# mfalt/FirstOrderSolvers.jl

Measured on AMD Instinct MI355X. Metric: GAP/DR outer iterations/sec (+ achieved HBM GB/s of the CG SpMV in `roofline`), higher is better.
Workload: dtype f64

## Files before the change

### firstordersolvers.jl_amd/_lib.py

```python
from __future__ import annotations

import ctypes as C
import os
from pathlib import Path

import numpy as np

_HERE = Path(__file__).resolve().parent
LIB_PATH = Path(os.environ["FOSHIP_LIB"]) if os.environ.get("FOSHIP_LIB") else _HERE / "csrc" / "libfoship.so"

FOS_OK = 0
CONE_CODES = {"Free": 0, "Zero": 1, "NonNeg": 2, "NonPos": 3, "SOC": 4, "SOCRotated": 5, "SDP": 6,
              "ExpPrimal": 7, "ExpDual": 8}
SET_CODES = {"IndFree": 0, "IndBallL2": 1, "IndBallL1": 2, "IndSimplex": 3, "IndHalfspace": 4, "IndHyperslab": 5, "IndPoint": 6, "IndBox": 7}
FN_CODES = {"NormL1": 32, "SqrNormL2": 33, "ElasticNet": 34, "Linear": 35, "NormL2": 36, "HuberLoss": 37, "NormLinf": 38}
LS_FORM_CODES = {"sparse_factored": 0, "normal": 1}
ALG_GAP, ALG_GAPA, ALG_FISTA, ALG_DYKSTRA = 0, 1, 2, 3
CG_REFERENCE, CG_FUSED_P, CG_MERGED_SWEEP, CG_MERGED_UPDATE, CG_RESIDENT = 0, 1, 2, 3, 4
DEBUG_PUPDATE_DELAY = 1
STATUS_NAMES = {0: "Continue", 1: "Optimal", 2: "Unbounded", 3: "Infeasible"}


class FosError(RuntimeError):
    def __init__(self, code, msg):
# ... 16 lines not shown
PROTOTYPES = {
    "fos_abi_version": (C.c_int, []),
    "fos_last_error": (C.c_char_p, []),
    "fos_device_count": (C.c_int, [_i32p]),
    "fos_device_name": (C.c_int, [C.c_int, C.c_char_p, C.c_int]),
    "fos_create": (C.c_int, [C.c_int64, C.c_int64, _i64p, _i64p, _dp, _dp, _dp,
                             C.c_int64, _i32p, _i64p, _i64p, C.c_int64, _i32p, _i64p, _i64p, C.c_int, C.POINTER(_h)]),
    "fos_create2": (C.c_int, [C.c_int64, C.c_int64, _i64p, _i64p, _dp, _dp, _dp,
                              C.c_int64, _i32p, _i64p, _i64p, C.c_int64, _i32p, _i64p, _i64p, C.c_int, C.c_int32, C.POINTER(_h)]),
    "fos_create3": (C.c_int, [C.c_int64, C.c_int64, _i64p, _i64p, _dp, _dp, _dp,
                              C.c_int64, _i32p, _i64p, _i64p, C.c_int64, _i32p, _i64p, _i64p, C.c_int, C.c_int32, C.c_int32, C.POINTER(_h)]),
    "fos_get_equilibration": (C.c_int, [_h, _i32p, _dp, _dp, _dp]),
    "fos_host_equilibrate": (C.c_int, [C.c_int64, C.c_int64, _i64p, _i64p, _dp, _dp, _dp,
                                       C.c_int64, _i32p, _i64p, _i64p, C.c_int64, _i32p, _i64p, _i64p, C.c_int32, _dp, _dp, _dp, _dp, _dp, _dp]),
    "fos_destroy": (C.c_int, [_h]),
    "fos_sizes": (C.c_int, [_h, _i64p, _i64p, _i64p, _i64p]),
    "fos_get_cg_total": (C.c_int, [_h, _i64p]),
    "fos_operator_stats": (C.c_int, [_h, _i64p]),
    "fos_comm_get_unique_id": (C.c_int, [C.c_void_p]),
    "fos_set_linesearch": (C.c_int, [_h, C.c_int64]),
    "fos_linesearch_log": (C.c_int, [_h, _dp]),
    "fos_set_longstep": (C.c_int, [_h, C.c_int64, C.c_int64]),
    "fos_longstep_log": (C.c_int, [_h, _dp]),
    "fos_comm_init": (C.c_int, [_h, C.c_int, C.c_int, C.c_void_p]),
    "fos_comm_init_host": (C.c_int, [_h, C.c_int, C.c_int, C.c_void_p, C.c_void_p]),
    "fos_peer_export": (C.c_int, [_h, C.c_void_p]),
    "fos_peer_open": (C.c_int, [_h, C.c_int, C.c_int, C.c_void_p, C.c_double]),
    "fos_peer_open_host": (C.c_int, [_h, C.c_int, C.c_int, C.c_char_p, C.c_double]),
    "fos_peer_close": (C.c_int, [_h]),
    "fos_peer_selftest": (C.c_int, [_h, C.c_int, C.POINTER(C.c_int32)]),
    "fos_exchange_bench": (C.c_int, [_h, C.c_int, _dp]),
    "fos_peer_vec_export": (C.c_int, [_h, C.c_void_p]),
    "fos_peer_vec_open": (C.c_int, [_h, C.c_void_p]),
    "fos_peer_enable": (C.c_int, [_h, C.c_int32]),
    "fos_set_alg": (C.c_int, [_h, C.c_int, C.c_double, C.c_double, C.c_double, C.c_double]),
    "fos_reset_affine": (C.c_int, [_h]),
    "fos_enable_direct": (C.c_int, [_h, _i64p, _i64p, _dp]),
    "fos_disable_direct": (C.c_int, [_h]),
    "fos_get_direct_mode": (C.c_int, [_h, _i32p]),
    "fos_enable_direct2": (C.c_int, [_h, _i64p, _i64p, _dp, C.c_int32]),
    "fos_get_direct_stats": (C.c_int, [_h, _dp]),
    "fos_enable_direct3": (C.c_int, [_h, _i64p, _i64p, _dp, C.c_int32, C.c_int32]),
    "fos_get_direct_stats2": (C.c_int, [_h, _dp]),
    "fos_dense_spd_inverse": (C.c_int, [C.c_int32, C.c_int64, _dp, _dp, C.c_int32, _dp]),
    "fos_host_chol_inverse": (C.c_int, [C.c_int64, _dp, _dp, _i64p]),
    "fos_host_reduced_symm": (C.c_int, [C.c_int64, _dp, _dp, _dp, _i32p]),
    "fos_set_iterate": (C.c_int, [_h, _dp]),
    "fos_get_iterate": (C.c_int, [_h, _dp]),
    "fos_get_checked": (C.c_int, [_h, _dp]),
    "fos_step": (C.c_int, [_h, C.c_int64, C.c_int64, C.c_int64, C.c_double, _i64p, _i32p, C.POINTER(CheckResult)]),
    "fos_getsol": (C.c_int, [_h, _dp, C.c_int32, C.c_double, C.POINTER(CheckResult)]),
    "fos_get_affine_state": (C.c_int, [_h, _dp, _i64p, _i32p]),
    "fos_set_affine_state": (C.c_int, [_h, _dp, C.c_int64]),
    "fos_get_alg_state": (C.c_int, [_h, _dp, _dp, _dp]),
    "fos_set_alg_state": (C.c_int, [_h, _dp, _dp, _dp]),
    "fos_get_cgiter": (C.c_int, [_h, _i64p]),
    "fos_get_alpha12": (C.c_int, [_h, _dp]),
    "fos_get_prox_count": (C.c_int, [_h, _i64p]),
    "fos_q_apply": (C.c_int, [_h, _dp, _dp, C.c_int32]),
    "fos_kkt_apply": (C.c_int, [_h, _dp, _dp]),
    "fos_cg_kkt": (C.c_int, [_h, _dp, _dp, C.c_double, C.c_int64, _i64p]),
    "fos_prox_affine": (C.c_int, [_h, _dp, _dp]),
    "fos_hsdematrix_prox": (C.c_int, [_h, _dp, _dp]),
    "fos_prox_cones": (C.c_int, [_h, _dp, _dp]),
    "fos_check": (C.c_int, [_h, _dp, C.c_double, C.POINTER(CheckResult)]),
    "fos_profile": (C.c_int, [_h, C.c_int32]),
    "fos_profile_read": (C.c_int, [_h, _i64p, _dp, _dp]),
    "fos_profile_read_classes": (C.c_int, [_h, _i64p, _dp]),
    "fos_bench_cg_chain": (C.c_int, [_h, C.c_int32, C.c_int32, C.c_int32, _dp]),
    "fos_bench_kkt": (C.c_int, [_h, C.c_int32, _dp]),
    "fos_psd_debug": (C.c_int, [_h, C.c_int32, C.c_int32]),
    "fos_psd_stats": (C.c_int, [_h, _i32p, C.c_int64, _i64p]),
    "fos_psd_fused_steps": (C.c_int, [_h, _i64p]),
    "fos_sync": (C.c_int, [_h]),
    "fos_host_stacked_spmv": (C.c_int, [C.c_int64, C.c_int64, _i64p, _i64p, _dp, _dp, _dp, C.c_int32, C.c_int32, _i64p]),
    "fos_host_resident_cg": (C.c_int, [C.c_int64, C.c_int64, _i64p, _i64p, _dp, _dp, _dp, C.c_int32, _dp, _dp, C.c_double, C.c_int64, _i64p, _i64p]),
    "fos_host_resident_plan": (C.c_int, [C.c_int64, C.c_int64, _i64p, _i64p, _dp, C.c_int32, _i64p, _i32p, C.c_int64, _i64p, C.c_int64]),
    "fos_host_stacked_spmv_mode": (C.c_int, [C.c_int64, C.c_int64, _i64p, _i64p, _dp, _dp, _dp, C.c_int32, _i64p]),
    "fos_window_stats": (C.c_int, [_h, _i64p]),
    "fos_set_tuning": (C.c_int, [_h, C.c_int32, C.c_int32, C.c_int32]),
    "fos_set_cg_variant": (C.c_int, [_h, C.c_int32]),
    "fos_get_cg_variant": (C.c_int, [_h, _i32p]),
    "fos_resident_stats": (C.c_int, [_h, _i64p]),
    "fos_debug_set": (C.c_int, [_h, C.c_int32, C.c_int64]),
    "fos_set_gapp": (C.c_int, [_h, C.c_int64]),
    "fos_gapp_log": (C.c_int, [_h, _dp]),
    "fos_feas_create": (C.c_int, [C.c_int64, C.c_int32, C.POINTER(_h)]),
    "fos_feas_destroy": (C.c_int, [_h]),
    "fos_feas_set_affine": (C.c_int, [_h, C.c_int32, C.c_int64, _dp, _dp]),
    "fos_feas_set_affine_sparse": (C.c_int, [_h, C.c_int32, C.c_int64, _i64p, _i64p, _dp, _dp]),
    "fos_feas_affine_stats": (C.c_int, [_h, C.c_int32, _dp]),
    "fos_feas_set_affine_factored": (C.c_int, [_h, C.c_int32, C.c_int64, _dp, _dp, C.c_int32, C.c_int32]),
    "fos_feas_affine_factored_stats": (C.c_int, [_h, C.c_int32, _dp]),
    "fos_feas_affine_factored_plan": (C.c_int, [_h, C.c_int32, _i64p]),
    "fos_host_affine_factored": (C.c_int, [C.c_int64, C.c_int64, _dp, _dp, C.c_int32, _dp, _dp]),
    "fos_feas_set_least_squares": (C.c_int, [_h, C.c_int32, C.c_int64, _dp, _dp, C.c_double, C.c_int32]),
    "fos_host_least_squares": (C.c_int, [C.c_int64, C.c_int64, _dp, _dp, C.c_double, _dp, _dp]),
    "fos_feas_set_affine_sparse_factored": (C.c_int, [_h, C.c_int32, C.c_int64, _i64p, _i64p, _dp, _dp, C.c_int32, C.c_int32]),
    "fos_feas_affine_sparse_factored_stats": (C.c_int, [_h, C.c_int32, _dp]),
    "fos_feas_affine_sparse_factored_plan": (C.c_int, [_h, C.c_int32, _i64p]),
    "fos_host_affine_sparse_factored": (C.c_int, [C.c_int64, C.c_int64, _i64p, _i64p, _dp, _dp, C.c_int32, _dp, _dp]),
    "fos_feas_set_quadratic": (C.c_int, [_h, C.c_int32, _dp, _dp, C.c_int32]),
    "fos_feas_set_least_squares_normal": (C.c_int, [_h, C.c_int32, C.c_int64, _dp, _dp, C.c_double, C.c_int32]),
    "fos_feas_set_least_squares_sparse": (C.c_int, [_h, C.c_int32, C.c_int64, _i64p, _i64p, _dp, _dp, C.c_double, C.c_int32, C.c_int32]),
    "fos_feas_nspace_stats": (C.c_int, [_h, C.c_int32, _dp]),
    "fos_host_quadratic": (C.c_int, [C.c_int64, _dp, _dp, _dp, _dp]),
    "fos_host_least_squares_normal": (C.c_int, [C.c_int64, C.c_int64, _dp, _dp, C.c_double, _dp, _dp]),
    "fos_host_least_squares_sparse": (C.c_int, [C.c_int64, C.c_int64, _i64p, _i64p, _dp, _dp, C.c_double, C.c_int32, _dp, _dp]),
    "fos_host_symv_packed": (C.c_int, [C.c_int64, _dp, _dp, _dp, _i32p]),
    "fos_feas_set_quadratic_sparse": (C.c_int, [_h, C.c_int32, _i64p, _i64p, _dp, _dp, C.c_double]),
    "fos_feas_set_least_squares_cg": (C.c_int, [_h, C.c_int32, C.c_int64, _i64p, _i64p, _dp, _dp, C.c_double, C.c_double]),
    "fos_feas_nspace_cg_stats": (C.c_int, [_h, C.c_int32, _dp]),
    "fos_host_quadratic_cg": (C.c_int, [C.c_int64, _i64p, _i64p, _dp, _dp, C.c_double, _dp, _dp, _i32p]),
    "fos_host_least_squares_cg": (C.c_int, [C.c_int64, C.c_int64, _i64p, _i64p, _dp, _dp, C.c_double, C.c_double, _dp, _dp, _i32p]),
    "fos_bench_symv_packed": (C.c_int, [C.c_int32, C.c_int64, C.c_int32, _dp]),
    "fos_feas_set_box": (C.c_int, [_h, C.c_int32, C.c_double, C.c_double]),
    "fos_feas_set_box_arrays": (C.c_int, [_h, C.c_int32, _dp, _dp]),
    "fos_feas_set_cones": (C.c_int, [_h, C.c_int32, C.c_int64, _i32p, _i64p]),
    "fos_feas_set_callback": (C.c_int, [_h, C.c_int32, C.c_void_p, C.c_void_p]),
    "fos_feas_set_blocks": (C.c_int, [_h, C.c_int32, C.c_int64, _i32p, _i64p, _dp, _dp]),
    "fos_feas_set_stats": (C.c_int, [_h, C.c_int32, _dp]),
    "fos_host_set_project": (C.c_int, [C.c_int32, C.c_int64, _dp, _dp, _dp, _dp, _i32p]),
    "fos_feas_set_alg": (C.c_int, [_h, C.c_int32, C.c_double, C.c_double, C.c_double, C.c_double]),
    "fos_feas_set_gapp": (C.c_int, [_h, C.c_double, C.c_double, C.c_double, C.c_int64]),
    "fos_feas_gapp_log": (C.c_int, [_h, _dp]),
    "fos_feas_set_linesearch": (C.c_int, [_h, C.c_int64]),
    "fos_feas_linesearch_log": (C.c_int, [_h, _dp]),
    "fos_feas_set_longstep": (C.c_int, [_h, C.c_int64, C.c_int64]),
    "fos_feas_longstep_log": (C.c_int, [_h, _dp]),
    "fos_feas_set_iterate": (C.c_int, [_h, _dp]),
    "fos_feas_step": (C.c_int, [_h, C.c_int64, C.c_int64, C.c_int64, C.c_double, _i64p, _i32p, _dp, _i32p]),
    "fos_feas_getsol": (C.c_int, [_h, _dp, C.c_int32, C.c_double, _i32p, _dp]),
    "fos_feas_get_iterate": (C.c_int, [_h, _dp]),
    "fos_feas_prox": (C.c_int, [_h, C.c_int32, _dp, _dp]),
    "fos_feas_info": (C.c_int, [_h, _dp, _i32p, _dp]),
}

_lib = None


def load(check_symbols=False):
    global _lib
    if _lib is not None and not check_symbols:
        return _lib
    if not LIB_PATH.exists():
        raise FosError(-100, "%s not found: build it with `make -C %s` (hipcc, gfx950); there is no CPU fallback"
                       % (LIB_PATH, LIB_PATH.parent))
    lib = C.CDLL(str(LIB_PATH), mode=getattr(os, "RTLD_NOW", 2) | getattr(os, "RTLD_GLOBAL", 0x100))
    for name, (res, args) in PROTOTYPES.items():
        fn = getattr(lib, name)
        fn.restype = res
        fn.argtypes = args
    if lib.fos_abi_version() != 1:
        raise FosError(-101, "ABI version mismatch")
    _lib = lib
    return lib


ALLREDUCE_FN = C.CFUNCTYPE(C.c_int, C.c_void_p, C.POINTER(C.c_double), C.c_int64)


def header_symbols():
    import re
    text = (_HERE.parent / "include" / "foship.h").read_text()
    text = re.sub(r"/\*.*?\*/", "", text, flags=re.S)
    return sorted(set(re.findall(r"\b(fos_[a-z0-9_]+)\s*\(", text)))
# ... 24 lines not shown
```

### firstordersolvers.jl_amd/csrc/fos_internal.hpp

```cpp
#pragma once

#include <hip/hip_runtime.h>

#include <algorithm>
#include <cstddef>
#include <cstdint>
#include <cstdio>
#include <cstring>
#include <string>
#include <vector>

#include "foship.h"

namespace fos {

void set_error(const char* fmt, ...);

#define FOS_HIP(expr)                                                                         \
    do {                                                                                      \
        hipError_t _e = (expr);                                                               \
        if (_e != hipSuccess) {                                                               \
            ::fos::set_error("%s:%d: %s -> %s", __FILE__, __LINE__, #expr, hipGetErrorString(_e)); \
            return FOS_EHIP;                                                                  \
        }                                                                                     \
// ... 244 lines not shown
    const PeerBox* fold;
    uint32_t seq_base;
    int32_t batch_mark = 0;
};
constexpr int CGM_RR_STRIDE = 1024;
void launch_cgm_sweep(const LaunchCtx& c, const CgmIter& it, int closes);
void launch_cgm_update(const LaunchCtx& c, const CgmIter& it, bool close_only);
void launch_cgm_apply(const LaunchCtx& c, const CgmIter& it, const double2* v);
void launch_cgm_start(const LaunchCtx& c, const CgmIter& it, const double2* rhs, const double2* v, double tol, int maxit,
                      double2* p_out = nullptr);

struct ResWG { int32_t blk0, nblk, c0, tc, T, wg0, wpu, idx; };
constexpr int RES_GMAX = 512;
constexpr int RES_WPU_MAX = 16;
constexpr int RES_SLOTS = 21;
constexpr int RS_GMAX = 256;
constexpr int RS_WPU_MAX = 4;
constexpr int RS_NCOMP = 7;
constexpr int RS_NTC = 6;
constexpr int RS_NTC_BASE = 3;
constexpr int RS_COMM_LEAD = 2;
inline int rs_ntc(int tmax) { return tmax > 32 ? RS_NTC_BASE : RS_NTC; }
__host__ __device__ inline void rs_split(uint32_t deal, int w, int& t0, int& cnt) {
    t0 = 0;
    for (int k = 0; k < w; ++k) t0 += (int)((deal >> (4 * k)) & 15u);
    cnt = (int)((deal >> (4 * w)) & 15u);
}
inline uint32_t rs_pack(const int (&cnt)[RS_NCOMP + 1]) {
    uint32_t deal = 0;
    for (int w = 0; w <= RS_NCOMP; ++w) deal |= (uint32_t)cnt[w] << (4 * w);
    return deal;
}
inline uint32_t rs_deal(int nblk, int ntc = RS_NTC) {
    int kc = std::min(nblk % RS_NCOMP, RS_NTC_BASE);
    for (int k = std::min(ntc, RS_NTC); k > kc; --k)
        if (k <= (nblk - k + RS_NCOMP - 1) / RS_NCOMP - RS_COMM_LEAD) { kc = k; break; }
    const int per = (nblk - kc) / RS_NCOMP, rem = (nblk - kc) % RS_NCOMP;
    int cnt[RS_NCOMP + 1];
    for (int w = 0; w < RS_NCOMP; ++w) cnt[w] = per + (w < rem ? 1 : 0);
    cnt[RS_NCOMP] = kc;
    return rs_pack(cnt);
}
inline bool rs_deal_ok(uint32_t deal, int nblk, int nt_cap, int ntc) {
    int sum = 0;
    bool gap = false;
    for (int w = 0, t0, cnt; w <= RS_NCOMP; ++w) {
        rs_split(deal, w, t0, cnt);
        if (cnt > (w < RS_NCOMP ? nt_cap : ntc)) return false;
        if (w < RS_NCOMP && cnt > 0 && gap) return false;
        if (cnt == 0) gap = true;
        sum += cnt;
    }
    return sum == nblk;
}
inline int rs_deal_nt(uint32_t deal) {
    int nt = 0;
    for (int w = 0, t0, cnt; w < RS_NCOMP; ++w) { rs_split(deal, w, t0, cnt); nt = std::max(nt, cnt); }
    return nt;
}
constexpr size_t RES_LDS_BUDGET = 160 * 1024;
constexpr size_t RS_STATIC_LDS_MAX = 2560;
inline size_t res_stream_lds_bytes(int tiles) {
    return (size_t)(RS_NCOMP + 1) * 64 * sizeof(double2) + (size_t)4 * RS_GMAX * sizeof(double) + (size_t)(RS_WPU_MAX - 1) * 64 * 2 * sizeof(double) +
           (size_t)tiles * 128 * sizeof(double2);
}
inline size_t res_reg_lds_bytes(int nslot, int tmax) {
    return (size_t)nslot * 64 * 4 * sizeof(double2) + (size_t)nslot * tmax * sizeof(double2) + (size_t)(RES_WPU_MAX - 1) * tmax * 2 * sizeof(double) +
           (size_t)4 * RES_GMAX * sizeof(double);
}
struct ResPlan {
    int G = 0, nw = 0, ncomm = 0, rpt = 0, tmax = 0, tiles_wg_max = 0, units = 0;
    int stream = 0, nt = 0;
    std::vector<ResWG> wg;
    std::string why;
};
bool build_resident_plan(const HostBlkCsr& S, int64_t m, int64_t n, int gmax, ResPlan* out);
int host_resident_cg(const HostBlkCsr& S, const ResPlan& P, int64_t m, int64_t n, const double* cb, double2* x, const double2* rhs, const double2* v0,
                     double tol, int maxit, int* iters);
struct ResLaunch {
    const ResWG* wg; int G, nw, ncomm, rpt, tmax, stream, nt, tiles_wg_max;
    unsigned long long* grec;
    unsigned long long* crec;
    int64_t timeout_ticks;
};
hipError_t launch_cg_resident(const LaunchCtx& c, const ResLaunch& rl, double2* x, const double2* rhs, const double2* v, double tol, int maxit,
                              const PeerBox* fold, uint32_t seq_base);
bool res_lds_fits(const ResLaunch& rl, int device, std::string* why);

enum QMode { Q_PLAIN = 0, Q_RHS = 1, Q_STATUS = 2, Q_VFROMU = 3, Q_PLAIN_NOTAU = 4 };
void launch_q1(const LaunchCtx& c, QMode mode, const double2* v, int comp, double sign, void* out);
void launch_q1_finalize(const LaunchCtx& c, QMode mode, const double2* v, int comp, double sign, void* out, int from_reduced);

void launch_cg_init(const LaunchCtx& c, const double2* rhs, const double2* Ap, double2* r, double2* p);
void launch_cg_init_finalize(const LaunchCtx& c, const double2* r, double tol, int maxit, int from_reduced);
void launch_reduce1(const LaunchCtx& c, int count, int nacc, int gate, int off = 0);
void launch_peer_chain(const LaunchCtx& c, int rounds);

constexpr int LONG_KMAX_ROWS = 32;
struct LongPlanes {
    int64_t interval = 0, nsave = 0;
    int64_t savepos = 0;
    bool now = false;
    double2* P = nullptr;
    double* bpart = nullptr;
    double* dots = nullptr;
    double* nu = nullptr;
    double log[8] = {0};
    int64_t max_supports = 4096;
};
struct LaunchCtx;
void long_save_plane(const LaunchCtx& c, LongPlanes& lp, int which, const double2* y, const double2* x);
int long_project_planes(const LaunchCtx& c, LongPlanes& lp, double2* X, int64_t i);
void launch_long_plane(const LaunchCtx& c, double2* row, const double2* x, const double2* y, double* bpart);
void launch_long_dots(const LaunchCtx& c, const double2* P, int K, int a, const double2* x, double* out);
void launch_long_apply(const LaunchCtx& c, double2* x, const double2* P, int K, const double* nu);
void launch_normdiff(const LaunchCtx& c, const double2* x, const double2* y);
void launch_shift_part2(const LaunchCtx& c, double2* out, const double2* y, const double2* x);
void launch_axpby(const LaunchCtx& c, double2* out, double a, const double2* x, double b, const double2* y);
void launch_relax_a12(const LaunchCtx& c, double2* out, const double2* y, const double2* x);
void launch_gap_final(const LaunchCtx& c, double2* x, const double2* t2, const double2* t1, double alpha, double alpha2,
                      double2* shift_out = nullptr, const double2* sol = nullptr);
void launch_gapa_final(const LaunchCtx& c, double2* x, const double2* t2, const double2* t1, double alpha,
                       double2* shift_out = nullptr, const double2* sol = nullptr);
void launch_gapa_finalize(const LaunchCtx& c, double beta, int from_reduced);
void launch_fista_extrap(const LaunchCtx& c, double2* y, const double2* x, const double2* xold, double coef);
void launch_add(const LaunchCtx& c, double2* out, const double2* a, const double2* b);
void launch_copy(const LaunchCtx& c, double2* out, const double2* in);
void launch_dykstra_corr(const LaunchCtx& c, double2* p, const double2* x, const double2* y);

void launch_dense_q_fill(const LaunchCtx& c, const int64_t* colptr, const int64_t* rowval, const double* nzval, double* Q, int64_t ld);
void launch_dense_gemm(const LaunchCtx& c, int L, double alpha, const double* A, const double* B, double gamma, const double* D, double* Cm);
void launch_dense_resid(const LaunchCtx& c, int64_t L, const double* Y, double* partials, int nblocks);
void launch_dense_scale_identity(const LaunchCtx& c, int64_t L, double* X, double s);
void launch_dense_symv(const LaunchCtx& c, int64_t ld, const double* G, const double* t, double* w);
void launch_dense_spd_inverse_chol(const LaunchCtx& c, int64_t L, const double* G, double* X, double* Lw, double* Ww, int32_t* info);
int64_t host_chol_inverse(int64_t k, const double* K, double* X, bool fused = false);
void launch_dense_gram_rows(const LaunchCtx& c, int64_t m, int64_t ld, const double* A, int64_t L, double* G);
void launch_direct_rhs(const LaunchCtx& c, const double2* W, const double2* x, double* t);
void launch_direct_finish(const LaunchCtx& c, const double2* x, const double2* W, double2* out);

constexpr int RED_TR = 64, RED_TC = 32;
constexpr int RED_TILE = RED_TR * RED_TC;
constexpr int RED_CHUNK = 16;
constexpr int RED_DOT_BLOCKS = 1024;
struct RedUnit { int32_t j, i0, i1, tile0; };
struct RedPlan {
    int64_t k = 0, ntiles = 0;
    int nt = 0, ns = 0;
    std::vector<RedUnit> units;
    std::vector<int32_t> strip_u0;
};
struct RedDev {
    int64_t k, kpad; int nt, nunits;
    const RedUnit* units; const int32_t* strip_u0;
    double* tiles;
    double2* rowslot;
    double* colslot;
};
void build_reduced_plan(int64_t k, RedPlan* P);
void host_reduced_pack(const RedPlan& P, const double* X, std::vector<double>* tiles, int32_t* count);
void host_reduced_symm(const RedPlan& P, const std::vector<double>& tiles, const double* pq, double* y);
void launch_red_form_k(const LaunchCtx& c, int64_t k, int64_t ld, const int32_t* cptr, const int32_t* cidx, const double* cval, const int32_t* rptr,
                       const int32_t* ridx, const double* rval, double* K);
void launch_red_pack_tiles(const LaunchCtx& c, const RedDev& R, int64_t ld, const double* X);
void launch_red_symm(const LaunchCtx& c, const RedDev& R, const double2* pq, double2* y);
void launch_red_in1(const LaunchCtx& c, int swap, const double* t, double2* vin);
void launch_red_pair(const LaunchCtx& c, const RedDev& R, int swap, const double* t, const double* s1, double2* pq);
// ... 230 lines not shown
```

### firstordersolvers.jl_amd/csrc/fos_solver.hpp

```cpp
#pragma once

#include <rccl/rccl.h>

#include <algorithm>

#include "fos_internal.hpp"

typedef double2 d2;

enum DirectForm : int32_t { DIRECT_OFF = 0, DIRECT_DENSE = 1, DIRECT_BLOCK = 2, DIRECT_CG = 3, DIRECT_REDUCED = 4 };

struct DenseInv {
    int used = FOS_DIRECT_FACTOR_NEWTON;
    int steps = 0;
    double seconds = 0.0, probe = 0.0;
    bool fell_back = false;
    int64_t bad_col = -1;
};

enum ReduceVia { VIA_NONE, VIA_RCCL, VIA_HOST, VIA_PEER };
struct HostSeg {
    void* p = nullptr;
    int fd = -1;
    size_t bytes = 0;
    std::string name;
    bool creator = false;
    volatile unsigned long long* ids() const { return reinterpret_cast<volatile unsigned long long*>(static_cast<char*>(p) + bytes - 4096); }
};
struct Transport {
    ncclComm_t comm = nullptr;
    fos_allreduce_fn host_fn = nullptr; void* host_user = nullptr;
    double* host_buf = nullptr;
    unsigned long long* peer_mbox = nullptr;
    unsigned long long* peer_relay = nullptr;
    std::vector<void*> peer_opened;
    fos::PeerBox peer{};
    bool peer_on{false};
    bool peer_same_device = false;
    HostSeg host_seg;
    double* vec_buf = nullptr;
    std::vector<void*> vec_opened;
    fos::VecBox vec{};
    uint32_t vec_seq = 0;
    ReduceVia via() const { return peer_on ? VIA_PEER : (host_fn ? VIA_HOST : (comm ? VIA_RCCL : VIA_NONE)); }
};

struct Operator {
    fos::HostBlkCsr host;
    fos::DevBlkCsr dev{};
    int32_t* wave_blk0 = nullptr; fos::BlkDesc* wave_first = nullptr;
    uint32_t* def_mask = nullptr;
    int64_t win_stats[4] = {0, 0, 0, 0};
    int nwg_target = 2048;
    double* slots_rd = nullptr;
    fos::DefRow* cmp_rec = nullptr; int32_t* cmp_idx = nullptr; double* cmp_local = nullptr; int cmp_lpr = 1;
    fos::ResPlan res_plan;
    fos::ResLaunch res{};
    fos::ResWG* res_wg = nullptr;
    bool res_ok = false;
    bool res_all = false;
    int res_gmax = 0;
};

struct fos_solver {
    int device = 0;
    hipStream_t stream = nullptr;
    int64_t m = 0, n = 0, l = 0, nnz = 0;
    int64_t l_global = 0;

    Operator op;
    std::vector<void*> owned;
    std::vector<void*> pooled;
    double* cb = nullptr;
    double nb = 0.0, nc = 0.0;
    double nb_local = 0.0, nc_local = 0.0;

    d2 *X = nullptr, *T1 = nullptr, *T2 = nullptr;
    d2 *SOL = nullptr, *RHS = nullptr, *R = nullptr, *AP = nullptr;
    d2 *PB[2] = {nullptr, nullptr};
    d2 *Y = nullptr, *XOLD = nullptr;
    d2 *W = nullptr;
    d2 *SOL2 = nullptr;
    double* plain = nullptr;

    fos::ConeSet* cones = nullptr;
    int cus = 256;
    bool psd_fuse = true;
    bool relax_ew = true;

    fos::DevState* st = nullptr;
    fos::DevState* st_host = nullptr;
    fos::HostMark* mark = nullptr;
    double* pre_sums = nullptr;
    bool pre_on = true;
    bool speculate = true;
    double* partials = nullptr;
    double* reduced = nullptr;
    int vec_blocks = 0;
    int cg_blocks = 0;
    bool fuse_p = false;
    int cg_variant = -1;

    int alg = FOS_ALG_GAP;
    double alpha = 0.8, alpha1 = 1.8, alpha2 = 1.8, beta = 0.0;
    double fista_t = 1.0;

    DirectForm direct_form = DIRECT_OFF;
    bool direct_exact() const { return direct_form != DIRECT_OFF && direct_form != DIRECT_CG; }
    double* Ginv = nullptr;
    int64_t Gld = 0;
    int direct_factor_req = 0;
    DenseInv direct_inv;
    double* dvec[2] = {nullptr, nullptr};
    int blk_n = 0;
    int64_t* blk_goff = nullptr;
    int32_t* blk_ioff = nullptr;
    int32_t* blk_idx = nullptr;
    double* blk_ginv = nullptr;
    d2 *blk_phg = nullptr, *blk_qphg = nullptr;
    double* blk_prm = nullptr;
    double* blk_ctx = nullptr;
    bool blk_skip_tail = true;
    bool blk_ready = false;
    bool red_ready = false;
    int red_swap = 0;
    int red_refine = 1;
    fos::RedPlan red_plan;
    fos::RedDev red{};
    d2 *red_pq = nullptr, *red_yk = nullptr;
    double *red_s = nullptr, *red_d = nullptr, *red_r = nullptr, *red_z = nullptr;
    double *red_p = nullptr, *red_q = nullptr, *red_g = nullptr;
    double* red_dots = nullptr;
    double red_minv[4] = {0, 0, 0, 0};
    double direct_setup_s = 0.0;

    int64_t prox_i = 1;
    bool firstrun = true;
    int64_t cgiter = 0;
    int hit_max_accum = 0;
    bool firstrun2 = true;
    int last_cg_pred = 0;
    bool shift_ready = false;
    bool shift_fuse = true;
    bool in_step = false;
    int64_t ls_interval = 0;
    bool ls_now = false;
    int64_t gapp_iproj = 0;
    bool gapp_now = false;
    double gapp_log[23] = {0};
    double ls_log[34] = {0};
    fos::LongPlanes lp;
    int cg_same_run = 0;
    const d2* last_checked = nullptr;

    Transport tr;
    int nranks = 1, rank = 0;
    uint32_t cg_epoch = 0;
    bool sharded() const { return tr.via() != VIA_NONE; }
    bool row_sharded = false;

    int eq_passes = 0;
    std::vector<double> eq_D, eq_E;
    double eq_sigma = 1.0, eq_rho = 1.0, eq_gamma = 1.0;
    double eq_nb = 0.0, eq_nc = 0.0;
    d2* eq_up = nullptr;
    double *eq_inv = nullptr, *eq_cb = nullptr, *eq_w = nullptr;
    bool equilibrated() const { return eq_passes > 0; }

    int cg_chunk = 8;
    bool prof = false;
    int prof_period = 1;
    int64_t cg_total = 0;
    int64_t direct_sweeps = 0;
    struct ProfRec { hipEvent_t a, b; int cls; int j; };
    std::vector<ProfRec> prof_recs;
    size_t prof_used = 0;
    int64_t prof_seen[FOS_PROF_CLASSES] = {0, 0, 0, 0, 0};
    int64_t prof_steps = 0, prof_steps_sampled = 0;
    bool prof_step_on = false;
    static constexpr size_t PROF_CAP = 16384;

    static int sum_slots_over_ranks(void* self);

    fos::LaunchCtx ctx(bool mailboxes = false) const {
        fos::LaunchCtx c;
        c.stream = stream; c.S = op.dev; c.cb = cb; c.n = n; c.m = m; c.l = l; c.st = st;
        c.partials = partials; c.reduced = reduced; c.vec_blocks = vec_blocks; c.cg_blocks = cg_blocks;
        c.peer = (tr.peer_on || mailboxes) ? &tr.peer : nullptr;
        c.def_mask = op.def_mask;
        c.pre = pre_on ? pre_sums : nullptr;
        c.between = nullptr; c.between_arg = nullptr;
        c.cus = cus;
        c.psd_refine_max_mats = (tr.peer_same_device && nranks > 1) ? std::max(1, cus / nranks) : 0;
        c.count_repl = (!row_sharded || rank == 0) ? 1 : 0;
        c.n_repl = row_sharded ? n : 0;
        if (row_sharded) { c.between = &fos_solver::sum_slots_over_ranks; c.between_arg = const_cast<fos_solver*>(this); }
        return c;
    }
};

namespace fos {
int allreduce(fos_solver* h, int count);
int finish_reduce(fos_solver* h, const LaunchCtx& c, int count, int nacc, int gate, int* from_reduced, int off = 0);
void transport_teardown(fos_solver* h, bool destroy = false);
bool peer_fold_env(), peer_loopback_env();
int global_setup(fos_solver* h);
int uncached_acquire(int device, size_t bytes, bool allow_plain, void** out, const char* what);
struct RoctxRange {
    bool on;
    explicit RoctxRange(const char* name);
    ~RoctxRange();
};
int check_launch(const char* where);
int prof_begin(fos_solver* h, int cls, int j, int64_t ordinal);
int prof_begin_other(fos_solver* h, int post);
void prof_end(fos_solver* h, int idx);
int poll_state(fos_solver* h);
int kkt_apply_full(fos_solver* h, const LaunchCtx& c, const d2* w, d2* out, bool deferred = true, bool tau_row = true);
int operator_setup(fos_solver* h, const int64_t* colptr, const int64_t* rowval, const double* nzval);
int operator_repartition(fos_solver* h, int nwg);
int resident_setup(fos_solver* h, int gmax);
int prox_affine_direct(fos_solver* h, const d2* x);

struct Scratch {
    std::vector<void*> held;
    hipError_t err = hipSuccess;
    Scratch() = default;
    Scratch(const Scratch&) = delete;
    Scratch& operator=(const Scratch&) = delete;
    ~Scratch() { for (void* p : held) (void)hipFree(p); }
    template <class T> T* alloc(size_t count) {
        void* p = nullptr;
        if (err == hipSuccess) err = hipMalloc(&p, sizeof(T) * count);
        if (err != hipSuccess) return nullptr;
        held.push_back(p);
        return static_cast<T*>(p);
    }
};

struct DenseWork {
    LaunchCtx c{};
    int64_t L = 0;
    double *G = nullptr, *B0 = nullptr, *B1 = nullptr, *B2 = nullptr, *v0 = nullptr, *v1 = nullptr, *partials = nullptr;
    void fill(Scratch& s) {
        const size_t L2 = (size_t)L * (size_t)L;
        for (double** b : {&B0, &B1, &B2}) *b = s.alloc<double>(L2);
        for (double** v : {&v0, &v1}) if (!*v) *v = s.alloc<double>((size_t)L);
        if (!partials) partials = s.alloc<double>(256);
    }
};
struct DenseOpts {
    const char *what, *gname;
    int factor;
    bool pivot_fallback;
    double bar = 1e-12;
    int newton_extra = 6;
};
int dense_spd_inverse(const DenseWork& k, const DenseOpts& o, double** Xout, DenseInv* st);
void direct_test_vector(int64_t k, int which, std::vector<double>& v);
int factored_inverse(const DevOwned& own, double lambda, int factor, double bar, hipStream_t stream, int64_t m, int64_t L, double* G, double* Xout, DenseInv* inv);

template <class Owner, class T>
int dev_alloc(Owner* h, T** p, size_t count) {
    void* q = nullptr;
    size_t bytes = std::max<size_t>(count, 1) * sizeof(T);
    hipError_t e = hipMalloc(&q, bytes);
    if (e != hipSuccess) { set_error("hipMalloc(%zu bytes): %s", bytes, hipGetErrorString(e)); return FOS_ENOMEM; }
    h->owned.push_back(q);
    *p = reinterpret_cast<T*>(q);
    return FOS_OK;
}

template <class Owner, class T>
int dev_zeros(Owner* h, T** p, size_t count) {
    FOS_TRY(dev_alloc(h, p, count));
    FOS_HIP(hipMemset(*p, 0, sizeof(T) * count));
    return FOS_OK;
}

template <class T>
void dev_release(fos_solver* h, T** p) {
    if (!*p) return;
    auto it = std::find(h->owned.begin(), h->owned.end(), (void*)*p);
    if (it != h->owned.end()) h->owned.erase(it);
    (void)hipFree(*p);
    *p = nullptr;
}

template <class Owner, class T>
int dev_upload(Owner* h, T** p, const std::vector<T>& v) {
    FOS_TRY(dev_alloc(h, p, v.size()));
    if (!v.empty()) FOS_HIP(hipMemcpy(*p, v.data(), v.size() * sizeof(T), hipMemcpyHostToDevice));
    return FOS_OK;
}

inline double sum_squares(const double* v, int64_t count) {
    double s = 0;
    for (int64_t i = 0; i < count; ++i) s += v[i] * v[i];
    return s;
}
}
```

### firstordersolvers.jl_amd/csrc/operator.cpp

```cpp
#include "fos_solver.hpp"

namespace fos {

static int first_target(int cus, const char* wg_env) {
    return wg_env ? std::max(1, std::min(16384, atoi(wg_env))) : cus * 12;
}

static int build_product_operator(int64_t m, int64_t n, const int64_t* colptr, const int64_t* rowval, const double* nzval, int cus, bool row_sharded,
                                  const char* wg_env, HostBlkCsr* out) {
    return build_stacked_csr(m, n, colptr, rowval, nzval, first_target(cus, wg_env), out, cus * 28, -1, row_sharded, cus * 16);
}

static int choose_sweep_grid(HostBlkCsr& hs, int cus, const char* wg_env) {
    int target = first_target(cus, wg_env);
    if (!hs.wpanel.empty()) {
        int nwg = std::min<int>((int)hs.wpanel.size(), cus * hs.wgeom.wg_per_cu);
        if (wg_env) nwg = std::max(1, std::min<int>(atoi(wg_env), (int)hs.wpanel.size()));
        if (nwg >= 8 && (int)hs.wpanel.size() > nwg) nwg -= nwg % 8;
        hs.nwg = nwg;
    } else if (!wg_env && hs.ntiles > hs.nblk / 2) {
        const int64_t waves_target = (int64_t)target * SPMV_WAVES;
        int64_t per_wave = std::max<int64_t>(1, (hs.nblk + waves_target / 2) / waves_target);
        while ((hs.nblk + SPMV_WAVES * per_wave - 1) / (SPMV_WAVES * per_wave) > 16384) ++per_wave;
        target = (int)((hs.nblk + SPMV_WAVES * per_wave - 1) / (SPMV_WAVES * per_wave));
// ... 77 lines not shown
        FOS_TRY(upload(h, &D.wval, hs.wval));
        FOS_TRY(upload(h, &D.wcol, hs.wcol));
        FOS_TRY(upload(h, &D.wrow, hs.wrow));
        window_stats4(hs, o.win_stats);
        drop(hs.wval); drop(hs.wcol); drop(hs.wrow);
    }
    D.nrows = hs.nrows; D.nnz = hs.nnz; D.nnz_padded = hs.nnz_padded;
    D.dbg_flags = getenv("FOS_DBG_FLAGS") ? atoi(getenv("FOS_DBG_FLAGS")) : 0;
    const double op_bytes = 8.0 * (double)hs.nnz_padded + 4.0 * (double)hs.ncol_stored + 48.0 * (double)hs.nblk;
    D.resident = (hs.wpanel.empty() && hs.ntiles == 0 && op_bytes <= 48e6) ? 1 : 0;
    if (const char* e = getenv("FOS_RESIDENT")) D.resident = atoi(e) != 0 ? 1 : 0;
    D.wave_blk0 = o.wave_blk0; D.wave_first = o.wave_first; D.nblk = hs.nblk; D.nwg = hs.nwg; D.nwaves = hs.nwaves;
    D.ndef = (int32_t)hs.def_rows.size(); D.def_lpr = 1;
    if (D.ndef > 0) {
        int32_t* ddi;
        FOS_TRY(upload(h, &D.row_defer, hs.row_defer));
        FOS_TRY(upload(h, &D.def_rows, hs.def_rows));
        FOS_TRY(upload(h, &D.def_ptr, hs.def_ptr));
        FOS_TRY(dev_upload(h, &ddi, hs.def_idx));
        double avg_list = (double)hs.def_ptr.back() / (double)D.ndef;
        if (!(h->row_sharded && hs.ntiles > 0)) {
            FOS_TRY(upload(h, &D.def_rec, hs.def_rec));
            FOS_TRY(dev_zeros(h, &D.slots, (size_t)2 * hs.nslots));
            D.slots_rd = D.slots; D.def_idx = ddi;
            if (h->row_sharded) {
                FOS_TRY(dev_zeros(h, &o.slots_rd, (size_t)2 * hs.nslots));
                D.slots_rd = o.slots_rd;
            }
        } else {
            const size_t nn = (size_t)h->n;
            if (hs.def_rows.size() < nn || hs.def_rows[nn - 1] != (int32_t)(nn - 1)) { set_error("internal: row-sharded tile operator without all rows of A' deferred"); return FOS_EINVAL; }
            TwoViews v;
            two_views(hs.def_rec, hs.def_idx, hs.def_ptr, nn, &v);
            FOS_TRY(dev_upload(h, &o.cmp_rec, v.cmp_rec));
            o.cmp_idx = ddi; o.cmp_lpr = lanes_per_row(v.cmp_avg);
            FOS_TRY(dev_zeros(h, &o.cmp_local, 2 * nn));
            FOS_TRY(upload(h, &D.def_rec, v.rec));
            FOS_TRY(upload(h, &D.def_idx, v.idx));
            FOS_TRY(dev_zeros(h, &o.slots_rd, 2 * (nn + (size_t)hs.nslots)));
            D.slots_rd = o.slots_rd; D.slots = o.slots_rd + 2 * nn;
            avg_list = v.avg;
        }
        int lpr = lanes_per_row(avg_list);
        if (getenv("FOS_DEF_LPR")) lpr = std::max(1, std::min(64, atoi(getenv("FOS_DEF_LPR"))));
        while (lpr & (lpr - 1)) lpr &= lpr - 1;
        D.def_lpr = lpr;
        D.nwg_def = (int32_t)std::min<int64_t>(DEF_MAX_WG, ((int64_t)D.ndef * lpr + DEF_THREADS - 1) / DEF_THREADS);
        std::vector<uint32_t> mask((size_t)(h->l + 31) / 32 + 1, 0u);
        for (int32_t r : hs.def_rows) mask[(size_t)r >> 5] |= 1u << (r & 31);
        FOS_TRY(dev_upload(h, &o.def_mask, mask));
        drop(hs.row_defer); drop(hs.def_idx);
    }
    set_parts(D);
    drop(hs.val); drop(hs.col); drop(hs.row_rel);
    return FOS_OK;
}

int operator_repartition(fos_solver* h, int nwg) {
    Operator& o = h->op;
    nwg = std::min(nwg, 16384);
    if (o.dev.npanel > 0) {
        o.dev.nwg = std::max(1, std::min<int32_t>(nwg, o.dev.npanel));
    } else {
        FOS_HIP(hipStreamSynchronize(h->stream));
        partition_workgroups(&o.host, nwg);
        FOS_HIP(hipMemcpy(o.wave_blk0, o.host.wave_blk0.data(), o.host.wave_blk0.size() * sizeof(int32_t), hipMemcpyHostToDevice));
        FOS_HIP(hipMemcpy(o.wave_first, o.host.wave_first.data(), o.host.wave_first.size() * sizeof(BlkDesc), hipMemcpyHostToDevice));
        o.dev.nwg = o.host.nwg; o.dev.nwaves = o.host.nwaves; o.nwg_target = nwg;
    }
    set_parts(o.dev);
    return FOS_OK;
}

static ResLaunch plan_launch(const ResPlan& p, ResLaunch rl) {
    rl.G = p.G; rl.nw = p.nw; rl.ncomm = p.ncomm; rl.rpt = p.rpt; rl.tmax = p.tmax; rl.stream = p.stream; rl.nt = p.nt; rl.tiles_wg_max = p.tiles_wg_max;
    return rl;
}

static void plan_stats8(const ResPlan& p, bool ok, bool all, int64_t* stats8) {
    stats8[0] = ok ? 1 : 0; stats8[1] = p.G; stats8[2] = p.nw; stats8[3] = p.stream ? -p.nt : p.rpt; stats8[4] = p.units; stats8[5] = p.tiles_wg_max;
    stats8[6] = p.tmax; stats8[7] = all ? 1 : 0;
}

int resident_setup(fos_solver* h, int gmax) {
    Operator& o = h->op;
    if (const char* e = getenv("FOS_RESIDENT_GMAX")) gmax = std::max(1, std::min(gmax, atoi(e)));
    if (o.res_gmax == gmax) return FOS_OK;
    o.res_gmax = gmax; o.res_ok = false;
    ResPlan plan;
    bool ok = build_resident_plan(o.host, h->m, h->n, gmax, &plan);
    if (ok) {
        std::string why;
        ok = res_lds_fits(plan_launch(plan, ResLaunch{}), h->device, &why);
        if (!ok) { plan.why = why; plan.G = 0; plan.wg.clear(); }
    }
    if (!ok) { o.res_plan = plan; o.res_all = false; return FOS_OK; }
    FOS_HIP(hipStreamSynchronize(h->stream));
    if (!o.res.grec) {
        constexpr size_t b1 = sizeof(unsigned long long) * 2 * RES_GMAX * 8, b2 = sizeof(unsigned long long) * 2 * RES_GMAX * 64 * 4;
        void *q1 = nullptr, *q2 = nullptr;
        FOS_TRY(uncached_acquire(h->device, b1, true, &q1, "resident CG records"));
        h->pooled.push_back(q1);
        FOS_TRY(uncached_acquire(h->device, b2, true, &q2, "resident CG column records"));
        h->pooled.push_back(q2);
        FOS_HIP(hipMemset(q1, 0, b1));
        FOS_HIP(hipMemset(q2, 0, b2));
        o.res.grec = static_cast<unsigned long long*>(q1); o.res.crec = static_cast<unsigned long long*>(q2);
    }
    dev_release(h, &o.res_wg);
    FOS_TRY(dev_upload(h, &o.res_wg, plan.wg));
    o.res.wg = o.res_wg;
    o.res = plan_launch(plan, o.res);
    static const double res_wait_s = getenv("FOS_RESIDENT_WAIT_S") ? atof(getenv("FOS_RESIDENT_WAIT_S")) : 5.0;
    o.res.timeout_ticks = (int64_t)(res_wait_s * 1e8);
    o.res_plan = plan; o.res_ok = true; o.res_all = !h->sharded();
    return FOS_OK;
}

static void format_stats12(const HostBlkCsr& S, int64_t* stats) {
    int64_t nell = 0, nlds = 0, nlong = 0, nrun = 0;
    for (const BlkDesc& d : S.blk) {
        if (d.kind() == BLK_ELL) ++nell; else if (d.kind() == BLK_LDS) ++nlds; else if (d.kind() == BLK_LONG) ++nlong;
        if (d.run()) ++nrun;
    }
    stats[0] = S.nblk; stats[1] = nell; stats[2] = nlds; stats[3] = nlong; stats[4] = nrun;
    stats[5] = S.nnz_padded; stats[6] = S.ncol_stored; stats[7] = S.nwaves;
    stats[8] = S.ntiles; stats[9] = S.nslots; stats[10] = (int64_t)S.def_rows.size(); stats[11] = S.tile_values;
}

}

using namespace fos;

extern "C" {

int fos_operator_stats(fos_handle h, int64_t* stats) {
    if (!h || !stats) { set_error("NULL argument"); return FOS_EINVAL; }
    format_stats12(h->op.host, stats);
    stats[7] = h->op.dev.nwaves; stats[10] = h->op.dev.ndef;
    return FOS_OK;
}

int fos_window_stats(fos_handle h, int64_t* stats4) {
    if (!h || !stats4) { set_error("NULL argument"); return FOS_EINVAL; }
    for (int k = 0; k < 4; ++k) stats4[k] = h->op.win_stats[k];
    return FOS_OK;
}

int fos_resident_stats(fos_handle h, int64_t* stats8) {
    if (!h || !stats8) { set_error("NULL argument"); return FOS_EINVAL; }
    const Operator& o = h->op;
    plan_stats8(o.res_plan, o.res_ok, h->sharded() ? o.res_all : o.res_ok, stats8);
    if (!o.res_ok) set_error("FOS_CG_RESIDENT: %s", o.res_plan.why.empty() ? "no plan" : o.res_plan.why.c_str());
    return FOS_OK;
}

int fos_host_resident_cg(int64_t m, int64_t n, const int64_t* colptr, const int64_t* rowval, const double* nzval, const double* b, const double* c,
                         int32_t gmax, double* x, const double* rhs, double tol, int64_t max_iters, int64_t* iters, int64_t* stats8) {
    if (!colptr || m < 0 || n < 0 || gmax < 1 || (x && (!rhs || !b || !c || max_iters < 1))) { set_error("bad argument"); return FOS_EINVAL; }
    HostBlkCsr S;
    FOS_TRY(build_product_operator(m, n, colptr, rowval, nzval, 256, false, nullptr, &S));
    ResPlan P;
    const bool ok = build_resident_plan(S, m, n, gmax, &P);
    if (stats8) plan_stats8(P, ok, ok, stats8);
    if (!ok) { set_error("FOS_CG_RESIDENT: the operator does not qualify (%s)", P.why.c_str()); return x ? FOS_EUNSUPPORTED : FOS_OK; }
    if (!x) return FOS_OK;
    const int64_t l = n + m + 1;
    std::vector<double> cb((size_t)(n + m));
    for (int64_t j = 0; j < n; ++j) cb[j] = c[j];
    for (int64_t i = 0; i < m; ++i) cb[n + i] = b[i];
    std::vector<double2> xv((size_t)l), rv((size_t)l);
    for (int64_t i = 0; i < l; ++i) { xv[i] = double2{x[i], x[l + i]}; rv[i] = double2{rhs[i], rhs[l + i]}; }
    std::vector<double2> v0(xv);
    int it = 0;
    FOS_TRY(host_resident_cg(S, P, m, n, cb.data(), xv.data(), rv.data(), v0.data(), tol, (int)std::min<int64_t>(max_iters, 1 << 30), &it));
    for (int64_t i = 0; i < l; ++i) { x[i] = xv[i].x; x[l + i] = xv[i].y; }
    if (iters) *iters = it;
    return FOS_OK;
}

int fos_host_resident_plan(int64_t m, int64_t n, const int64_t* colptr, const int64_t* rowval, const double* nzval, int32_t gmax,
                           int64_t* info8, int32_t* wg7, int64_t wg_cap, int64_t* tile5, int64_t tile_cap) {
    if (!colptr || !info8 || m < 0 || n < 0 || gmax < 1) { set_error("bad argument"); return FOS_EINVAL; }
    HostBlkCsr S;
    FOS_TRY(build_product_operator(m, n, colptr, rowval, nzval, 256, false, nullptr, &S));
    ResPlan P;
    const bool ok = build_resident_plan(S, m, n, gmax, &P);
    int64_t ntiles = 0;
    for (const ResWG& w : P.wg) ntiles += w.nblk;
    info8[0] = ok ? (P.stream ? 2 : 1) : 0; info8[1] = P.G; info8[2] = P.nt; info8[3] = P.tmax; info8[4] = P.nw; info8[5] = P.rpt; info8[6] = P.ncomm;
    info8[7] = ntiles;
    if (!ok) { set_error("FOS_CG_RESIDENT: the operator does not qualify (%s)", P.why.c_str()); return FOS_OK; }
    if (wg7 && wg_cap >= P.G)
        for (int q = 0; q < P.G; ++q) {
            const ResWG& w = P.wg[q];
            const int32_t r[7] = {w.blk0, w.nblk, w.c0, w.tc, w.wg0, w.wpu, w.idx};
            memcpy(wg7 + 7 * (size_t)q, r, sizeof(r));
        }
    if (tile5 && tile_cap >= ntiles) {
        int64_t k = 0;
        for (const ResWG& w : P.wg)
            for (int ti = 0; ti < w.nblk; ++ti, ++k) {
                const BlkDesc& d = S.blk[w.blk0 + ti];
                int64_t* t = tile5 + 5 * k;
                t[0] = d.meta[0]; t[1] = d.meta[3]; t[2] = d.steps(); t[3] = d.nrows(); t[4] = d.row0;
            }
    }
    return FOS_OK;
}

int fos_debug_resident_deal(int32_t tiles, int32_t steps, int32_t* cnt8, int64_t* lds_bytes) {
    if (tiles < 0 || steps < 1 || steps > 64 || !cnt8) { set_error("bad argument"); return FOS_EINVAL; }
    const uint32_t deal = rs_deal(tiles, rs_ntc(steps));
    for (int w = 0, t0, cnt; w <= RS_NCOMP; ++w) { rs_split(deal, w, t0, cnt); cnt8[w] = cnt; }
    if (lds_bytes) *lds_bytes = (int64_t)res_stream_lds_bytes(tiles);
    return FOS_OK;
}

int fos_host_stacked_spmv(int64_t m, int64_t n, const int64_t* colptr, const int64_t* rowval, const double* nzval,
                          const double* v, double* out, int32_t spmv_workgroups, int32_t resident_waves, int64_t* stats) {
    if (!colptr || !v || !out || m < 0 || n < 0) { set_error("bad argument"); return FOS_EINVAL; }
    HostBlkCsr S;
    FOS_TRY(build_stacked_csr(m, n, colptr, rowval, nzval, spmv_workgroups > 0 ? spmv_workgroups : 1024, &S, resident_waves));
    std::string why;
    int rc = host_stacked_spmv(S, v, out, &why);
    if (rc != FOS_OK) { set_error("operator format check failed: %s", why.c_str()); return rc; }
    if (stats) format_stats12(S, stats);
    return FOS_OK;
}

int fos_host_stacked_spmv_mode(int64_t m, int64_t n, const int64_t* colptr, const int64_t* rowval, const double* nzval,
                               const double* v, double* out, int32_t window_mode, int64_t* stats16) {
    if (!colptr || !v || !out || m < 0 || n < 0) { set_error("bad argument"); return FOS_EINVAL; }
    HostBlkCsr S;
    const bool rs = getenv("FOS_HOST_SPMV_ROW_SHARDED") && atoi(getenv("FOS_HOST_SPMV_ROW_SHARDED")) != 0;
    FOS_TRY(build_stacked_csr(m, n, colptr, rowval, nzval, 1024, &S, 0, window_mode, rs));
// ... 13 lines not shown
```

### firstordersolvers.jl_amd/csrc/resident.hip

```cpp
#include "dev_common.hpp"

namespace fos {

struct ResArgs {
    d2* x;
    const d2* rhs;
    const d2* v;
    const double* cb;
    int n, nm;
    DevState* st;
    const BlkDesc* blk;
    const double* val;
    const ResWG* wg;
    int G;
    unsigned long long* grec;
    unsigned long long* crec;
    int tmax;
    int ncomp;
    int flags;
    double tol;
    int maxit;
    PeerBox pb;
    uint32_t seq_base;
    long long timeout_ticks;
};

__device__ __forceinline__ void res_st_word(unsigned long long* p, unsigned long long w) { __hip_atomic_store(p, w, __ATOMIC_RELAXED, __HIP_MEMORY_SCOPE_AGENT); }
__device__ __forceinline__ unsigned long long res_ld_word(const unsigned long long* p) { return __hip_atomic_load(p, __ATOMIC_RELAXED, __HIP_MEMORY_SCOPE_AGENT); }
__device__ __forceinline__ void res_publish_half(unsigned long long* p, uint32_t seq, double v, int hh) {
    const unsigned long long bits = (unsigned long long)__double_as_longlong(v);
    res_st_word(p + hh, ((unsigned long long)seq << 32) | (hh ? (bits >> 32) : (bits & 0xFFFFFFFFull)));
}
__device__ __forceinline__ bool res_poll_f64(const unsigned long long* p, uint32_t seq, long long timeout, double& out) {
    const long long t0 = wall_clock64();
    unsigned long long lo, hi;
    bool ok;
    do {
        lo = res_ld_word(p); hi = res_ld_word(p + 1);
        ok = (uint32_t)(lo >> 32) == seq && (uint32_t)(hi >> 32) == seq;
    } while (!ok && (wall_clock64() - t0) < timeout);
    out = __longlong_as_double((long long)((hi << 32) | (lo & 0xFFFFFFFFull)));
    return ok;
}

template <int TMAX>
__device__ __forceinline__ void res_tile(const double (&val)[TMAX], int T, const d2 g, const char* __restrict__ gcol, const int (&xoff)[TILE_GROUP],
                                         d2* __restrict__ colpart, int lane, double& u1, double& u2) {
    u1 = 0.0; u2 = 0.0;
#pragma unroll
    for (int grp = 0; grp < TMAX / TILE_GROUP; ++grp) {
        if (grp * TILE_GROUP < T) {
            double p[TILE_GROUP];
#pragma unroll
            for (int h = 0; h < 2; ++h) {
#pragma unroll
                for (int u = 4 * h; u < 4 * h + 4; ++u) {
                    const d2 xc = *reinterpret_cast<const d2*>(gcol + grp * TILE_GROUP * (int)sizeof(d2) + xoff[u]);
                    u1 += val[grp * TILE_GROUP + u] * xc.x; u2 += val[grp * TILE_GROUP + u] * xc.y;
                    p[u] = val[grp * TILE_GROUP + u] * g.x;
                }
                __builtin_amdgcn_sched_barrier(0);
            }
            const double s1 = tile_colsum8_sorted(p);
            __builtin_amdgcn_sched_barrier(0);
#pragma unroll
            for (int u = 0; u < TILE_GROUP; ++u) p[u] = val[grp * TILE_GROUP + u] * g.y;
            const double s2 = tile_colsum8_sorted(p);
            if (lane < TILE_GROUP) colpart[grp * TILE_GROUP + lane] = make_double2(s1, s2);
            __builtin_amdgcn_sched_barrier(0);
        }
    }
}

#ifdef FOS_RES_STAMPS
__device__ long long g_res_stamps[4 * 16 * 64 * 16];
#define RES_STAMP(ph) do { if (stamp_slot >= 0 && stamp_it < 62 && (threadIdx.x & 63) == 0) { __builtin_amdgcn_sched_barrier(0); g_res_stamps[((size_t)stamp_slot * 64 + stamp_it) * 16 + (ph)] = (long long)__builtin_readcyclecounter(); __builtin_amdgcn_sched_barrier(0); } } while (0)
#define RES_STAMP_CAL(where) do { if (stamp_slot >= 0 && (threadIdx.x & 63) == 0) { g_res_stamps[((size_t)stamp_slot * 64 + (where)) * 16 + 6] = (long long)__builtin_readcyclecounter(); g_res_stamps[((size_t)stamp_slot * 64 + (where)) * 16 + 7] = wall_clock64(); } } while (0)
#define RES_STAMP_NEXT() do { stamp_it += 1; } while (0)
#else
#define RES_STAMP(ph) do { } while (0)
#define RES_STAMP_CAL(where) do { } while (0)
#define RES_STAMP_NEXT() do { } while (0)
#endif

enum ResCtl { RC_ALPHA = 0, RC_BETA, RC_GTX, RC_GTY, RC_STOP, RC_NEAR, RC_COUNT };

__device__ __forceinline__ bool res_peer_fold4(const PeerBox& pb, uint32_t seq, double (&tot)[4], bool first, uint32_t* halves ) {
    const int lane = threadIdx.x & 63;
    const size_t par = (size_t)((((seq >> 11) & 1u) << 1) | (seq & 1u)) * PEER_MAX_RANKS;
    bool bad = false;
    for (int t = lane; t < pb.nranks * 8; t += 64) {
        const int hh = t & 1, v = (t >> 1) & 3, r = t >> 3;
        const double mine_d = v == 0 ? tot[0] : (v == 1 ? tot[1] : (v == 2 ? tot[2] : tot[3]));
        const unsigned long long bits = (unsigned long long)__double_as_longlong(mine_d);
        const uint32_t mine = hh ? (uint32_t)(bits >> 32) : (uint32_t)bits;
        if (r == pb.rank && !pb.loopback) { halves[t] = mine; continue; }
        const size_t off_in = PEER_BOX_WORDS + ((par + r) * PEER_MAX_VALS + v) * 2 + hh;
        if (first) {
            const bool wr = !pb.shared || pb.loopback ? (r != pb.rank || pb.loopback) : (r == (pb.rank == 0 ? 1 : 0));
            if (wr) {
                unsigned long long* dst = pb.box[r] + PEER_BOX_WORDS + ((par + pb.rank) * PEER_MAX_VALS + v) * 2 + hh;
                __hip_atomic_store(dst, ((unsigned long long)seq << 32) | mine, __ATOMIC_RELAXED, __HIP_MEMORY_SCOPE_SYSTEM);
            }
        }
        const bool via_relay = pb.relay != nullptr && !first;
        const unsigned long long* src = via_relay ? pb.relay + off_in : pb.box[pb.rank] + off_in;
        long long t0 = 0;
        unsigned long long w;
        bool ok;
        for (uint32_t spin = 1;; ++spin) {
            w = __hip_atomic_load(src, __ATOMIC_RELAXED, __HIP_MEMORY_SCOPE_SYSTEM);
            ok = (uint32_t)(w >> 32) == seq;
            if (ok) break;
            if ((spin & 255u) == 0u) {
                const long long now = wall_clock64();
                if (t0 == 0) t0 = now;
                else if (now - t0 >= pb.timeout_ticks) break;
            }
        }
        if (!ok) bad = true;
        else if (pb.relay != nullptr && first) __hip_atomic_store(pb.relay + off_in, w, __ATOMIC_RELAXED, __HIP_MEMORY_SCOPE_SYSTEM);
        halves[t] = (uint32_t)w;
    }
    __builtin_amdgcn_fence(__ATOMIC_RELEASE, "wavefront");
    __builtin_amdgcn_wave_barrier();
    __builtin_amdgcn_fence(__ATOMIC_ACQUIRE, "wavefront");
    if (__builtin_amdgcn_ballot_w64(bad) != 0ull) return false;
#pragma unroll
    for (int v = 0; v < 4; ++v) {
        double sacc = 0.0;
        for (int r = 0; r < pb.nranks; ++r) {
            const unsigned long long lo = halves[(r * 4 + v) * 2], hi = halves[(r * 4 + v) * 2 + 1];
            sacc += __longlong_as_double((long long)((hi << 32) | lo));
        }
        tot[v] = sacc;
    }
    __builtin_amdgcn_fence(__ATOMIC_RELEASE, "wavefront");
    __builtin_amdgcn_wave_barrier();
    return true;
}

template <int TMAX, int RPT, int LB>
__global__ __launch_bounds__(LB) void cg_resident_kernel(ResArgs a) {
    __shared__ __attribute__((aligned(16))) d2 s_gcol[TMAX];
    __shared__ double s_red[16][4];
    __shared__ double s_ctl[RC_COUNT];
    __shared__ uint32_t s_halves[PEER_MAX_RANKS * 8];
    __shared__ int s_cnt, s_failed;
    extern __shared__ __attribute__((aligned(16))) double s_dyn[];
    constexpr int NSLOT = (LB / 64) * RPT;
    d2* const s_x = reinterpret_cast<d2*>(s_dyn);
    d2* const s_p = s_x + NSLOT * 64;
    d2* const s_s = s_p + NSLOT * 64;
    d2* const s_w = s_s + NSLOT * 64;
    d2* const s_colpart = s_w + NSLOT * 64;
    double* const s_sib = reinterpret_cast<double*>(s_colpart + NSLOT * TMAX);
    double* const s_all = s_sib + (RES_WPU_MAX - 1) * TMAX * 2;
    const int tid = threadIdx.x, lane = tid & 63;
    const int wv = __builtin_amdgcn_readfirstlane(tid >> 6), nw = (int)(blockDim.x >> 6);
    const int ncomp = a.ncomp, ncomm = nw - ncomp;
    const ResWG me = a.wg[blockIdx.x];
    const int T = me.T, tc = me.tc, c0 = me.c0, nm = a.nm;
    DevState* st = a.st;
#ifdef FOS_RES_STAMPS
    int stamp_slot = -1, stamp_it = 0;
    {
        const int b = (int)blockIdx.x;
        const int wslot = b == 0 ? 0 : (b == 1 ? 1 : (b == a.G / 2 ? 2 : (b == a.G - 1 ? 3 : -1)));
// ... 285 lines not shown
#pragma unroll
                for (int k = 0; k < 4; ++k) {
                    const int si = k < me.idx ? k : k - 1;
                    d2 part = k == me.idx ? cp : (si == 0 ? sv[0] : (si == 1 ? sv[1] : (si == 2 ? sv[2] : sv[3])));
                    if (k >= me.wpu) part = make_double2(0.0, 0.0);
                    t.x += part.x; t.y += part.y;
                }
                for (int k = 4; k < me.wpu; ++k) {
                    d2 part = cp;
                    if (k != me.idx) { const int si = k < me.idx ? k : k - 1; part = sib[(size_t)si * TMAX + lane]; }
                    t.x += part.x; t.y += part.y;
                }
                ctot = t;
            }
            const double q1 = ctot.x + gt.x * cc, q2 = ctot.y + gt.y * cc;
            const d2 cwv = make_double2(cr.x - q2, q1 - cr.y);
            const d2 wt = make_double2(gt.x + tot[3], -tot[2] - gt.y);
            RES_STAMP(12);
            double stopf = failed ? 2.0 : 0.0, alpha = 0.0, beta = 0.0;
            if (!failed) {
                if (i < 0) {
                    cr = make_double2(crhs.x - cwv.x, crhs.y - cwv.y);
                    gt = make_double2(rhst.x - wt.x, rhst.y - wt.y);
                } else {
                    gam = tot[0] + (gt.x * gt.x + gt.y * gt.y);
                    if (i > 0 && (sqrt(gam) <= a.tol || i >= a.maxit)) { iter = i; stopf = 1.0; }
                    else {
                        const double delta = tot[1] + (wt.x * gt.x + wt.y * gt.y);
                        if (i == 0) alpha = gam / delta;
                        else {
                            beta = gam / g_prev;
                            alpha = gam / (delta - beta * gam / a_prev);
                        }
                        g_prev = gam; a_prev = alpha;
                        auto upd = [&](const d2 wi, d2& ri, d2& pi, d2& si, d2& xi) {
                            if (i == 0) { pi = ri; si = wi; }
                            else {
                                pi.x = pi.x * beta + ri.x; pi.y = pi.y * beta + ri.y;
                                si.x = si.x * beta + wi.x; si.y = si.y * beta + wi.y;
                            }
                            xi.x += alpha * pi.x; xi.y += alpha * pi.y;
                            ri.x -= alpha * si.x; ri.y -= alpha * si.y;
                        };
                        if (lane < tc) upd(cwv, cr, cpv, csv, cx);
                        upd(wt, gt, pt, stt, xt);
                    }
                }
            }
            RES_STAMP(13);
            if (stopf == 0.0) {
                colG = (leader && lane < tc) ? cr.x * cr.x + cr.y * cr.y : 0.0;
                if (lane < tc) s_gcol[lane] = cr;
            }
            if (lane == 0) { s_ctl[RC_ALPHA] = alpha; s_ctl[RC_BETA] = beta; s_ctl[RC_GTX] = gt.x; s_ctl[RC_GTY] = gt.y; s_ctl[RC_STOP] = stopf; }
        }
        RES_STAMP(6);
        __syncthreads();
        RES_STAMP(7);
        RES_STAMP_NEXT();
        RES_STAMP(0);
        if (s_ctl[RC_STOP] != 0.0) break;
    }
    RES_STAMP_CAL(62);
    if (c0wave) {
        const bool ok = s_ctl[RC_STOP] == 1.0;
        if (ok && leader && lane < tc) a.x[c0 + lane] = cx;
        if (blockIdx.x == 0 && lane == 0) {
            if (ok) {
                a.x[nm] = xt;
                st->rr = gam;
                cg_signal_stop(st, iter, a.maxit, gam, a.seq_base >> 11);
            } else {
                if (a.pb.nranks > 0) st->xchg_failed = 1;
                st->bar_failed = 1; st->done = 1;
            }
        }
    }
}


#ifndef RS_XC
#define RS_XC 2
#endif
__device__ __forceinline__ void res_tile_plain(const double (&val)[TILE_GROUP], const d2 g, const d2* __restrict__ gcol, d2& u, double (&a1)[TILE_GROUP],
                                               double (&a2)[TILE_GROUP]) {
#pragma unroll
    for (int h = 0; h < TILE_GROUP / RS_XC; ++h) {
        d2 xc[RS_XC];
#pragma unroll
        for (int k = 0; k < RS_XC; ++k) xc[k] = gcol[RS_XC * h + k];
#pragma unroll
        for (int k = 0; k < RS_XC; ++k) {
            const double v = val[RS_XC * h + k];
            u.x += v * xc[k].x; u.y += v * xc[k].y;
            a1[RS_XC * h + k] += v * g.x; a2[RS_XC * h + k] += v * g.y;
        }
        __builtin_amdgcn_sched_barrier(0);
    }
}

__device__ __forceinline__ BlkDesc rs_desc(const BlkDesc* blk, int i) {
    typedef const __attribute__((address_space(4))) int64_t cs64;
    cs64* p = (cs64*)(blk + i);
    const int64_t w3 = p[3], w4 = p[4], w5 = p[5];
    BlkDesc d;
    d.nnz0 = p[0]; d.colpos = p[1]; d.cnt = p[2];
    d.row0 = (int32_t)w3; d.info = (int32_t)(w3 >> 32);
    d.meta[0] = (int32_t)w4; d.meta[1] = (int32_t)(w4 >> 32); d.meta[2] = (int32_t)w5; d.meta[3] = (int32_t)(w5 >> 32);
    return d;
}

__device__ __forceinline__ void rs_request(const ResArgs& a, int blk, int grp, int lane, double (&val)[TILE_GROUP]) {
    const BlkDesc d = rs_desc(a.blk, blk);
    const bool live = TILE_GROUP * grp < d.steps();
    const double* __restrict__ vp = a.val + d.nnz0 + (live ? 64 * TILE_GROUP * grp : 0) + (live ? lane : 0);
#pragma unroll
    for (int t = 0; t < TILE_GROUP; ++t) val[t] = __builtin_nontemporal_load(vp + 64 * t);
}


template <int NT> struct RsRows { d2 rr[NT], ww[NT], xx[NT]; };

template <int NT>
__device__ __forceinline__ void rs_rows_load(const ResArgs& a, int blk_first, int cnt, int lane, RsRows<NT>& R) {
#pragma unroll
    for (int q = 0; q < NT; ++q) {
        R.rr[q] = R.ww[q] = R.xx[q] = make_double2(0.0, 0.0);
        if (q < cnt) {
            const BlkDesc d = rs_desc(a.blk, blk_first + q);
            if (lane < d.nrows()) { R.rr[q] = a.v[d.row0 + lane]; R.xx[q] = a.x[d.row0 + lane]; }
        }
    }
}
template <int NT>
__device__ __forceinline__ void rs_rows_store(const ResArgs& a, int blk_first, int cnt, int lane, const RsRows<NT>& R) {
#pragma unroll
    for (int q = 0; q < NT; ++q) {
        if (q < cnt) {
            const BlkDesc d = rs_desc(a.blk, blk_first + q);
            if (lane < d.nrows()) a.x[d.row0 + lane] = R.xx[q];
        }
    }
}

template <int Q, int NT, int D>
__device__ __forceinline__ void rs_group(const ResArgs& a, int bf, int cnt, int grp, int c0, int lane, const d2* __restrict__ s_gcol, d2* __restrict__ mycol,
                                         RsRows<NT>& R, double (&val)[D][TILE_GROUP], double (&a1)[TILE_GROUP], double (&a2)[TILE_GROUP]) {
    if constexpr (Q < NT) {
        if (Q < cnt) {
            const BlkDesc d = rs_desc(a.blk, bf + Q);
            const int coff = d.meta[0] - c0 + TILE_GROUP * grp;
            const bool in = TILE_GROUP * grp < d.steps();
            if (in) res_tile_plain(val[Q % D], R.rr[Q], s_gcol + coff, R.ww[Q], a1, a2);
            if (Q + D < NT && Q + D < cnt) rs_request(a, bf + Q + D, grp, lane, val[Q % D]);
            else rs_request(a, bf + Q % D, grp + 1, lane, val[Q % D]);
            const bool last = Q + 1 == NT || Q + 1 >= cnt || rs_desc(a.blk, bf + Q + 1).meta[0] != d.meta[0];
            if (in && last) {
                const double s1 = tile_colsum8(a1, lane);
                const double s2 = tile_colsum8(a2, lane);
                if (lane < TILE_GROUP && TILE_GROUP * grp + lane < d.meta[3]) mycol[coff + lane] = make_double2(s1, s2);
#pragma unroll
                for (int u = 0; u < TILE_GROUP; ++u) a1[u] = a2[u] = 0.0;
            }
            rs_group<Q + 1, NT, D>(a, bf, cnt, grp, c0, lane, s_gcol, mycol, R, val, a1, a2);
        }
    }
}

#ifndef RS_RING
#define RS_RING 2
#endif
template <int TMAX, int NT>
__device__ __forceinline__ void rs_sweep(const ResArgs& a, int blk_first, int cnt, int c0, int lane, const d2* __restrict__ s_gcol, const double* s_ctl,
                                         d2* __restrict__ mycol, RsRows<NT>& R, double (&acc)[4], bool early = false,
                                         const double* __restrict__ cbh = nullptr) {
    constexpr int D = NT < RS_RING ? NT : RS_RING;
    if (early) cnt = 0;
    mycol[lane] = make_double2(0.0, 0.0);
    acc[0] = acc[1] = acc[2] = acc[3] = 0.0;
    if (cnt > 0) {
        int tw = 0;
#pragma unroll
        for (int q = 0; q < NT; ++q) { const int t = rs_desc(a.blk, blk_first + (q < cnt ? q : cnt - 1)).steps(); tw = t > tw ? t : tw; }
        const int ngrp = ((tw < TMAX ? tw : TMAX) + TILE_GROUP - 1) / TILE_GROUP;
        double val[D][TILE_GROUP], a1[TILE_GROUP], a2[TILE_GROUP];
#pragma unroll
        for (int s = 0; s < D; ++s) if (s < cnt) rs_request(a, blk_first + s, 0, lane, val[s]);
#pragma unroll
        for (int q = 0; q < NT; ++q) R.ww[q] = make_double2(0.0, 0.0);
#pragma unroll
        for (int u = 0; u < TILE_GROUP; ++u) a1[u] = a2[u] = 0.0;
        for (int grp = 0; grp < ngrp; ++grp) {
            int bf = blk_first;
            asm volatile("" : "+s"(bf));
            rs_group<0, NT, D>(a, bf, cnt, grp, c0, lane, s_gcol, mycol, R, val, a1, a2);
        }
        double cb[NT];
#pragma unroll
        for (int q = 0; q < NT; ++q) {
            cb[q] = 0.0;
            if (cbh) cb[q] = cbh[q];
            else if (q < cnt) {
                const BlkDesc d = rs_desc(a.blk, blk_first + q);
                if (lane < d.nrows()) cb[q] = a.cb[d.row0 + lane];
            }
        }
        const d2 gt = make_double2(s_ctl[RC_GTX], s_ctl[RC_GTY]);
#pragma unroll
        for (int q = 0; q < NT; ++q) {
            if (q < cnt) {
                const bool valid = lane < rs_desc(a.blk, blk_first + q).nrows();
                const d2 gq = R.rr[q];
                const double c = cb[q], u1 = R.ww[q].x, u2 = R.ww[q].y;
                const double q1 = -(u1 - gt.x * c), q2 = -(u2 - gt.y * c);
                d2 w = make_double2(gq.x - q2, q1 - gq.y);
                if (!valid) w = make_double2(0.0, 0.0);
                R.ww[q] = w;
                acc[2] += c * gq.x;
                acc[3] += c * gq.y;
            }
        }
    }
#pragma unroll
    for (int q = 0; q < NT; ++q) {
        acc[0] += R.rr[q].x * R.rr[q].x + R.rr[q].y * R.rr[q].y;
        acc[1] += R.ww[q].x * R.rr[q].x + R.ww[q].y * R.rr[q].y;
    }
    if (early) acc[1] = 0.0;
}

template <int NT>
__device__ __forceinline__ void rs_update(const ResArgs& a, int blk_first, int slot_first, int cnt, int lane, int i, double alpha, double beta,
                                          d2* __restrict__ s_ps, RsRows<NT>& R) {
#pragma unroll
    for (int q = 0; q < NT; ++q) {
        if (q < cnt) {
            const size_t e = (size_t)(slot_first + q) * 128 + lane;
            const d2 w = R.ww[q];
            if (i < 0) {
                const BlkDesc d = a.blk[blk_first + q];
                const d2 rh = lane < d.nrows() ? a.rhs[d.row0 + lane] : make_double2(0.0, 0.0);
                R.rr[q] = make_double2(rh.x - w.x, rh.y - w.y);
            } else {
                d2 pq, sq;
                if (i == 0) { pq = R.rr[q]; sq = w; }
                else {
                    pq = s_ps[e]; sq = s_ps[e + 64];
                    pq.x = pq.x * beta + R.rr[q].x; pq.y = pq.y * beta + R.rr[q].y;
                    sq.x = sq.x * beta + w.x; sq.y = sq.y * beta + w.y;
                }
                R.xx[q].x += alpha * pq.x; R.xx[q].y += alpha * pq.y;
                R.rr[q].x -= alpha * sq.x; R.rr[q].y -= alpha * sq.y;
                s_ps[e] = pq; s_ps[e + 64] = sq;
            }
        }
        if ((q & 1) == 1) __builtin_amdgcn_sched_barrier(0);
    }
}

__device__ __forceinline__ bool rs_poll(const ResArgs& a, const ResWG& me, unsigned long long* grec, size_t par, uint32_t seq, int t, int nthr,
                                        double* __restrict__ s_all, double* __restrict__ s_sib) {
    const int tc = me.tc;
    const int nrec = 4 * a.G, nsib = (me.wpu - 1) * tc * 2;
    const int sleepn = (a.flags >> 8) & 0x7F;
    constexpr int PU = 3;
    bool bad = false;
    for (int base = t; base < nrec + nsib; base += PU * nthr) {
        const unsigned long long* src[PU];
        double* dst[PU];
#pragma unroll
        for (int u = 0; u < PU; ++u) {
            const int idx = base + u * nthr;
            src[u] = nullptr; dst[u] = nullptr;
            if (idx < nrec) {
                const int wg = idx >> 2, kk = idx & 3;
                dst[u] = s_all + (size_t)kk * RS_GMAX + wg;
                src[u] = wg == (int)blockIdx.x ? nullptr : grec + (size_t)wg * 8 + 2 * kk;
            } else if (idx < nrec + nsib) {
                const int j = idx - nrec, comp = j & 1, c = (j >> 1) % tc, si = (j >> 1) / tc;
                const int kk = si < me.idx ? si : si + 1;
                dst[u] = s_sib + ((size_t)si * 64 + c) * 2 + comp;
                src[u] = a.crec + ((par * a.G + (size_t)(me.wg0 + kk)) * (size_t)a.tmax + (size_t)c) * 4 + 2 * comp;
            }
        }
        long long tstart = 0;
        for (uint32_t spin = 1;; ++spin) {
            unsigned long long lo[PU], hi[PU];
#pragma unroll
            for (int u = 0; u < PU; ++u) if (src[u]) { lo[u] = res_ld_word(src[u]); hi[u] = res_ld_word(src[u] + 1); }
            bool pending = false;
#pragma unroll
            for (int u = 0; u < PU; ++u) {
                if (src[u]) {
                    if ((uint32_t)(lo[u] >> 32) == seq && (uint32_t)(hi[u] >> 32) == seq) {
                        *dst[u] = __longlong_as_double((long long)((hi[u] << 32) | (lo[u] & 0xFFFFFFFFull)));
                        src[u] = nullptr;
                    } else pending = true;
                }
            }
            if (!pending) break;
            if ((spin & 255u) == 0u) {
                const long long now = wall_clock64();
                if (tstart == 0) tstart = now;
                else if (now - tstart >= a.timeout_ticks) { bad = true; break; }
            }
            if (sleepn >= 2) __builtin_amdgcn_s_sleep(2); else if (sleepn >= 1) __builtin_amdgcn_s_sleep(1);
        }
    }
    return !bad;
}

template <int TMAX, int NT>
__global__ __launch_bounds__(64 * (RS_NCOMP + 1)) void cg_stream_kernel(ResArgs a) {
    __shared__ __attribute__((aligned(16))) d2 s_gcol[64];
    __shared__ double s_red[16][4];
    __shared__ double s_ctl[RC_COUNT];
    __shared__ uint32_t s_halves[PEER_MAX_RANKS * 8];
    __shared__ int s_cnt, s_failed;
    __shared__ double s_tau[9];
    extern __shared__ __attribute__((aligned(16))) double s_dyn[];
    d2* const s_colpart = reinterpret_cast<d2*>(s_dyn);
    double* const s_all = reinterpret_cast<double*>(s_colpart + (RS_NCOMP + 1) * 64);
    double* const s_sib = s_all + 4 * RS_GMAX;
    d2* const s_ps = reinterpret_cast<d2*>(s_sib + (RS_WPU_MAX - 1) * 64 * 2);
    const int tid = threadIdx.x, lane = tid & 63;
    const int wv = __builtin_amdgcn_readfirstlane(tid >> 6), nw = (int)(blockDim.x >> 6);
    constexpr int ncomp = RS_NCOMP;
    const int ncomm = nw - ncomp;
    const ResWG me = a.wg[blockIdx.x];
    const int tc = me.tc, c0 = me.c0, nm = a.nm;
    DevState* st = a.st;
#ifdef FOS_RES_STAMPS
    int stamp_slot = -1, stamp_it = 0;
    {
        const int b = (int)blockIdx.x;
        const int wslot = b == 0 ? 0 : (b == 1 ? 1 : (b == a.G / 2 ? 2 : (b == a.G - 1 ? 3 : -1)));
        if (wslot >= 0 && wv < 16) stamp_slot = wslot * 16 + wv;
    }
#endif
    if (a.pb.nranks > 0 && st->xchg_failed) return;
    if (tid == 0) { s_cnt = 0; s_failed = 0; }
    RES_STAMP_CAL(63);
#ifdef FOS_RES_STAMPS
    if (stamp_slot >= 0 && lane == 0) g_res_stamps[((size_t)stamp_slot * 64 + 63) * 16 + 5] = (long long)__builtin_amdgcn_s_getreg((31 << 11) | 4);
#endif
    int t0, cnt;
    rs_split((uint32_t)me.T, wv, t0, cnt);

    if (wv < ncomp) {
        RsRows<NT> R;
        rs_rows_load<NT>(a, me.blk0 + t0, cnt, lane, R);
        constexpr bool HOLD_CB = NT <= 9;
        double cbh[NT];
#pragma unroll
        for (int q = 0; q < NT; ++q) {
            cbh[q] = 0.0;
            if (HOLD_CB && q < cnt) {
                const BlkDesc d = rs_desc(a.blk, me.blk0 + t0 + q);
                if (lane < d.nrows()) cbh[q] = a.cb[d.row0 + lane];
            }
        }
        d2* const mycol = s_colpart + wv * 64;
        __syncthreads();
        RES_STAMP(0);
        bool early = false;
        for (int i = -1, xr = 0;; ++xr) {
            double acc[4];
            rs_sweep<TMAX, NT>(a, me.blk0 + t0, cnt, c0, lane, s_gcol, s_ctl, mycol, R, acc, early, HOLD_CB ? cbh : nullptr);
#pragma unroll
            for (int k = 0; k < 4; ++k) {
                const double v = wave_sum(acc[k]);
                if (lane == 0) s_red[wv][k] = v;
            }
            RES_STAMP(1);
            __syncthreads();
            RES_STAMP(2);
            {
                const uint32_t seq = a.seq_base + (uint32_t)(xr + 1);
                const size_t par = (size_t)(seq & 1u);
                if (!rs_poll(a, me, a.grec + par * (size_t)a.G * 8, par, seq, tid, (int)blockDim.x, s_all, s_sib)) s_failed = 1;
                __builtin_amdgcn_fence(__ATOMIC_RELEASE, "workgroup");
                if (lane == 0) __hip_atomic_fetch_add(&s_cnt, 1, __ATOMIC_RELAXED, __HIP_MEMORY_SCOPE_WORKGROUP);
            }
            __syncthreads();
            RES_STAMP(3);
            if (s_ctl[RC_STOP] != 0.0) break;
            if (!early) {
                rs_update<NT>(a, me.blk0 + t0, t0, cnt, lane, i, s_ctl[RC_ALPHA], s_ctl[RC_BETA], s_ps, R);
                early = s_ctl[RC_NEAR] != 0.0;
                ++i;
            } else early = false;
            RES_STAMP(4);
            RES_STAMP_NEXT();
            RES_STAMP(0);
        }
        if (s_ctl[RC_STOP] == 1.0) rs_rows_store<NT>(a, me.blk0 + t0, cnt, lane, R);
        RES_STAMP_CAL(62);
        return;
    }

    const int cw = wv - ncomp, ct = tid - 64 * ncomp;
    const bool c0wave = cw == 0, leader = me.idx == 0;
    d2 cx = make_double2(0.0, 0.0), cpv = cx, csv = cx;
    double cc = 0.0;
    for (int q = ct; q < 4 * RS_GMAX; q += 64 * ncomm) s_all[q] = 0.0;
    for (int q = ct + (ncomp + 1) * 4; q < 16 * 4; q += 64 * ncomm) (&s_red[0][0])[q] = 0.0;
    constexpr int NTC = TMAX > 32 ? RS_NTC_BASE : RS_NTC;
    RsRows<NTC> R;
    rs_rows_load<NTC>(a, me.blk0 + t0, c0wave ? cnt : 0, lane, R);
    d2* const mycol = s_colpart + ncomp * 64;
    if (c0wave) {
        d2 cr = make_double2(0.0, 0.0);
        if (lane < tc) { cr = a.v[c0 + lane]; cx = a.x[c0 + lane]; cc = a.cb[c0 + lane]; }
        s_gcol[lane] = cr;
        const d2 gt = a.v[nm], xt = a.x[nm];
        if (lane == 0) { s_ctl[RC_GTX] = gt.x; s_ctl[RC_GTY] = gt.y; s_ctl[RC_STOP] = 0.0; }
        if (lane == 0) { s_tau[0] = xt.x; s_tau[1] = xt.y; s_tau[2] = s_tau[3] = s_tau[4] = s_tau[5] = s_tau[6] = s_tau[7] = s_tau[8] = 0.0; }
        if (blockIdx.x == 0 && lane == 0) { st->tol = a.tol; st->maxit = a.maxit; st->hit_max = 0; st->rn_old = 0.0; }
    }
    __syncthreads();
    int iter = 0;
    uint32_t nx = 0;
    RES_STAMP(0);
    bool early = false;
    for (int i = -1, xr = 0;; ++xr) {
        const uint32_t seq = a.seq_base + (uint32_t)(xr + 1);
        const size_t par = (size_t)(seq & 1u);
        unsigned long long* grec = a.grec + par * (size_t)a.G * 8;
        nx += 1;
        if (c0wave) {
            double racc[4];
            rs_sweep<TMAX, NTC>(a, me.blk0 + t0, cnt, c0, lane, s_gcol, s_ctl, mycol, R, racc, early);
#pragma unroll
            for (int k = 0; k < 4; ++k) {
                const double v = wave_sum(racc[k]);
                if (lane == 0) s_red[ncomp][k] = v;
            }
        }
        RES_STAMP(14);
        __syncthreads();
        RES_STAMP(1);
        d2 cp = make_double2(0.0, 0.0);
        d2 gt = make_double2(0.0, 0.0), cr = gt, crhs = gt, rhst = gt;
        double colG = 0.0;
        if (c0wave) {
            gt = make_double2(s_ctl[RC_GTX], s_ctl[RC_GTY]);
            cr = s_gcol[lane];
            if (i < 0) { crhs = lane < tc ? a.rhs[c0 + lane] : make_double2(0.0, 0.0); rhst = a.rhs[nm]; }
            {
                double rx = cr.x, ry = cr.y;
                asm volatile("" : "+v"(rx), "+v"(ry));
                colG = (leader && lane < tc) ? rx * rx + ry * ry : 0.0;
            }
            double acc[4] = {0.0, 0.0, 0.0, 0.0};
            {
                d2 o[ncomp + 1];
#pragma unroll
                for (int s = 0; s < ncomp + 1; ++s) o[s] = s_colpart[s * 64 + lane];
#pragma unroll
                for (int s = 0; s < ncomp + 1; ++s) { cp.x += o[s].x; cp.y += o[s].y; }
            }
            if (lane < tc && early) { if (leader) acc[0] = colG; }
            else if (lane < tc) {
                acc[1] = cp.x * cr.y - cp.y * cr.x;
                if (leader) {
                    acc[0] = colG;
                    acc[1] += (cr.x * cr.x - cr.y * cr.y) + cc * (gt.x * cr.y - gt.y * cr.x);
                    acc[2] = cc * cr.x;
                    acc[3] = cc * cr.y;
                }
            }
            double mine[4];
            {
                double rv[12];
                const int k4 = lane & 3;
#pragma unroll
                for (int w = 0; w < 12; ++w) rv[w] = s_red[w][k4];
                double sacc = 0.0;
#pragma unroll
                for (int w = 0; w < 12; ++w) sacc += rv[w];
#pragma unroll
                for (int k = 0; k < 4; ++k) {
                    const int lo = __builtin_amdgcn_readlane(__double2loint(sacc), k), hi = __builtin_amdgcn_readlane(__double2hiint(sacc), k);
                    mine[k] = __hiloint2double(hi, lo) + wave_sum(acc[k]);
                }
            }
            if (i < 0) mine[0] = 0.0;
            if (early) { mine[1] = 0.0; mine[2] = 0.0; mine[3] = 0.0; }
            if (lane < 8) {
                const int k = lane >> 1;
                res_publish_half(grec + (size_t)blockIdx.x * 8 + 2 * k, seq, k == 0 ? mine[0] : (k == 1 ? mine[1] : (k == 2 ? mine[2] : mine[3])), lane & 1);
            }
            if (lane < 4) s_all[(size_t)lane * RS_GMAX + blockIdx.x] = lane == 0 ? mine[0] : (lane == 1 ? mine[1] : (lane == 2 ? mine[2] : mine[3]));
            if (me.wpu > 1 && lane < tc) {
                unsigned long long* p = a.crec + ((par * a.G + blockIdx.x) * (size_t)a.tmax + (size_t)lane) * 4;
                res_publish_half(p, seq, cp.x, 0); res_publish_half(p, seq, cp.x, 1);
                res_publish_half(p + 2, seq, cp.y, 0); res_publish_half(p + 2, seq, cp.y, 1);
            }
        }
        RES_STAMP(2);
        {
            if (!rs_poll(a, me, grec, par, seq, tid, (int)blockDim.x, s_all, s_sib)) s_failed = 1;
            __builtin_amdgcn_fence(__ATOMIC_RELEASE, "workgroup");
            if (lane == 0) __hip_atomic_fetch_add(&s_cnt, 1, __ATOMIC_RELAXED, __HIP_MEMORY_SCOPE_WORKGROUP);
        }
        RES_STAMP(3);
        if (c0wave) {
            {
                long long tstart = 0;
                for (uint32_t spin = 1; __hip_atomic_load(&s_cnt, __ATOMIC_RELAXED, __HIP_MEMORY_SCOPE_WORKGROUP) < (int)(nx * (uint32_t)nw); ++spin) {
                    if ((spin & 4095u) == 0u) {
                        const long long now = wall_clock64();
                        if (tstart == 0) tstart = now;
                        else if (now - tstart >= 2 * a.timeout_ticks) { s_failed = 1; break; }
                    }
                }
                __builtin_amdgcn_fence(__ATOMIC_ACQUIRE, "workgroup");
            }
            RES_STAMP(4);
            bool failed = __hip_atomic_load(&s_failed, __ATOMIC_RELAXED, __HIP_MEMORY_SCOPE_WORKGROUP) != 0;
            d2 xt = make_double2(s_tau[0], s_tau[1]), pt = make_double2(s_tau[2], s_tau[3]), stt = make_double2(s_tau[4], s_tau[5]);
            double g_prev = s_tau[6], a_prev = s_tau[7], gam = s_tau[8];
            double tot[4];
#pragma unroll
            for (int k = 0; k < 4; ++k) {
                double rv[RS_GMAX / 64];
#pragma unroll
                for (int j = 0; j < RS_GMAX / 64; ++j) rv[j] = s_all[(size_t)k * RS_GMAX + lane + 64 * j];
                double sacc = 0.0;
#pragma unroll
                for (int j = 0; j < RS_GMAX / 64; ++j) sacc += rv[j];
                tot[k] = wave_sum(sacc);
            }
            if (!failed && a.pb.nranks > 0) failed = !res_peer_fold4(a.pb, seq, tot, blockIdx.x == 0, s_halves);
            RES_STAMP(5);
            d2 ctot = cp;
            if (me.wpu > 1 && lane < tc) {
                const d2* sib = reinterpret_cast<const d2*>(s_sib);
                d2 t = make_double2(0.0, 0.0);
                for (int kk = 0; kk < me.wpu; ++kk) {
                    d2 part = cp;
                    if (kk != me.idx) part = sib[(size_t)(kk < me.idx ? kk : kk - 1) * 64 + lane];
                    t.x += part.x; t.y += part.y;
                }
                ctot = t;
            }
            const double q1 = ctot.x + gt.x * cc, q2 = ctot.y + gt.y * cc;
            const d2 cwv = make_double2(cr.x - q2, q1 - cr.y);
            const d2 wt = make_double2(gt.x + tot[3], -tot[2] - gt.y);
            double stopf = failed ? 2.0 : 0.0, alpha = 0.0, beta = 0.0, near = 0.0;
            if (!failed && early) {
                gam = tot[0] + (gt.x * gt.x + gt.y * gt.y);
                if (i > 0 && (sqrt(gam) <= a.tol || i >= a.maxit)) { iter = i; stopf = 1.0; }
            } else if (!failed) {
                if (i < 0) {
                    cr = make_double2(crhs.x - cwv.x, crhs.y - cwv.y);
                    gt = make_double2(rhst.x - wt.x, rhst.y - wt.y);
                } else {
                    gam = tot[0] + (gt.x * gt.x + gt.y * gt.y);
                    if (i > 0 && (sqrt(gam) <= a.tol || i >= a.maxit)) { iter = i; stopf = 1.0; }
                    else {
                        const double delta = tot[1] + (wt.x * gt.x + wt.y * gt.y);
                        if (i == 0) alpha = gam / delta;
                        else {
                            beta = gam / g_prev;
                            alpha = gam / (delta - beta * gam / a_prev);
                        }
                        g_prev = gam; a_prev = alpha;
                        auto upd = [&](const d2 wi, d2& ri, d2& pi, d2& si, d2& xi) {
                            if (i == 0) { pi = ri; si = wi; }
                            else {
                                pi.x = pi.x * beta + ri.x; pi.y = pi.y * beta + ri.y;
                                si.x = si.x * beta + wi.x; si.y = si.y * beta + wi.y;
                            }
                            xi.x += alpha * pi.x; xi.y += alpha * pi.y;
                            ri.x -= alpha * si.x; ri.y -= alpha * si.y;
                        };
                        if (lane < tc) upd(cwv, cr, cpv, csv, cx);
                        upd(wt, gt, pt, stt, xt);
                        near = (sqrt(gam) <= 3.0 * a.tol || i + 1 >= a.maxit) ? 1.0 : 0.0;
                    }
                }
            }
            if (stopf == 0.0 && !early) s_gcol[lane] = lane < tc ? cr : make_double2(0.0, 0.0);
            if (lane == 0) {
                if (!early) { s_ctl[RC_ALPHA] = alpha; s_ctl[RC_BETA] = beta; s_ctl[RC_GTX] = gt.x; s_ctl[RC_GTY] = gt.y; s_ctl[RC_NEAR] = near; }
                s_ctl[RC_STOP] = stopf;
                s_tau[0] = xt.x; s_tau[1] = xt.y; s_tau[2] = pt.x; s_tau[3] = pt.y; s_tau[4] = stt.x; s_tau[5] = stt.y; s_tau[6] = g_prev; s_tau[7] = a_prev; s_tau[8] = gam;
            }
        }
        RES_STAMP(6);
        __syncthreads();
        RES_STAMP(7);
        RES_STAMP_NEXT();
        RES_STAMP(0);
        if (s_ctl[RC_STOP] != 0.0) break;
        if (!early) {
            if (c0wave) rs_update<NTC>(a, me.blk0 + t0, t0, cnt, lane, i, s_ctl[RC_ALPHA], s_ctl[RC_BETA], s_ps, R);
            early = s_ctl[RC_NEAR] != 0.0;
            ++i;
        } else early = false;
    }
    RES_STAMP_CAL(62);
    if (c0wave) {
        const bool ok = s_ctl[RC_STOP] == 1.0;
        if (ok) rs_rows_store<NTC>(a, me.blk0 + t0, cnt, lane, R);
        if (ok && leader && lane < tc) a.x[c0 + lane] = cx;
        if (blockIdx.x == 0 && lane == 0) {
            if (ok) {
                a.x[nm] = make_double2(s_tau[0], s_tau[1]);
                const double gam = s_tau[8];
                st->rr = gam;
                cg_signal_stop(st, iter, a.maxit, gam, a.seq_base >> 11);
            } else {
                if (a.pb.nranks > 0) st->xchg_failed = 1;
                st->bar_failed = 1; st->done = 1;
            }
        }
    }
}

struct ResKernel { const void* fn; int threads; size_t lds; };
static ResKernel res_kernel(const ResLaunch& rl) {
    auto k = [](auto kern, int threads, size_t lds) { return ResKernel{reinterpret_cast<const void*>(kern), threads, lds}; };
    if (rl.stream) {
        const int thr = 64 * (RS_NCOMP + 1);
        const size_t lds = res_stream_lds_bytes(rl.tiles_wg_max);
        if (rl.tmax > 32 && rl.nt <= 3) return k(cg_stream_kernel<64, 3>, thr, lds);
        if (rl.tmax > 32) return k(cg_stream_kernel<64, 5>, thr, lds);
        if (rl.nt <= 3) return k(cg_stream_kernel<32, 3>, thr, lds);
        if (rl.nt <= 5) return k(cg_stream_kernel<32, 5>, thr, lds);
        if (rl.nt <= 9) return k(cg_stream_kernel<32, 9>, thr, lds);
        return k(cg_stream_kernel<32, 10>, thr, lds);
    }
    const int thr = 64 * (rl.nw + rl.ncomm);
    if (rl.tmax <= 32 && rl.rpt == 1) return k(cg_resident_kernel<32, 1, 768>, thr, res_reg_lds_bytes(12, 32));
    if (rl.tmax <= 32 && rl.rpt == 2) return k(cg_resident_kernel<32, 2, 512>, thr, res_reg_lds_bytes(16, 32));
    if (rl.tmax <= 32) return k(cg_resident_kernel<32, 3, 512>, thr, res_reg_lds_bytes(24, 32));
    return k(cg_resident_kernel<64, 1, 512>, thr, res_reg_lds_bytes(8, 64));
}

static hipError_t res_lds_optin(const ResKernel& k) {
    if (k.lds > 48 * 1024) return hipFuncSetAttribute(k.fn, hipFuncAttributeMaxDynamicSharedMemorySize, (int)k.lds);
    return hipSuccess;
}

bool res_lds_fits(const ResLaunch& rl, int device, std::string* why) {
    const ResKernel k = res_kernel(rl);
    hipFuncAttributes fa{};
    int cap = 0;
    char buf[192];
    if (hipFuncGetAttributes(&fa, k.fn) != hipSuccess || hipDeviceGetAttribute(&cap, hipDeviceAttributeMaxSharedMemoryPerBlock, device) != hipSuccess) {
        (void)hipGetLastError();
        *why = "the kernel's or the device's LDS size could not be read";
        return false;
    }
    if (k.lds + fa.sharedSizeBytes > (size_t)cap) {
        snprintf(buf, sizeof(buf), "a workgroup's LDS (%zu + %zu static bytes) exceeds the device's %d", k.lds, (size_t)fa.sharedSizeBytes, cap);
        *why = buf;
        return false;
    }
    const hipError_t e = res_lds_optin(k);
    if (e != hipSuccess) {
        (void)hipGetLastError();
        snprintf(buf, sizeof(buf), "the LDS opt-in for %zu bytes failed (%s)", k.lds, hipGetErrorString(e));
        *why = buf;
        return false;
    }
    return true;
}

hipError_t launch_cg_resident(const LaunchCtx& c, const ResLaunch& rl, double2* x, const double2* rhs, const double2* v, double tol, int maxit,
                              const PeerBox* fold, uint32_t seq_base) {
    ResArgs a{};
    a.x = x; a.rhs = rhs; a.v = v; a.cb = c.cb; a.n = (int)c.n; a.nm = (int)(c.n + c.m); a.st = c.st;
    a.blk = c.S.blk; a.val = c.S.val; a.wg = rl.wg; a.G = rl.G; a.grec = rl.grec; a.crec = rl.crec; a.tmax = rl.tmax;
    a.tol = tol; a.maxit = maxit;
    a.pb = fold ? *fold : PeerBox{}; a.seq_base = seq_base;
    a.timeout_ticks = rl.timeout_ticks;
    a.ncomp = rl.nw;
    static const int res_flags = getenv("FOS_RES_FLAGS") ? atoi(getenv("FOS_RES_FLAGS")) : (2 << 8);
    a.flags = res_flags;
    const ResKernel k = res_kernel(rl);
    const hipError_t e = res_lds_optin(k);
    if (e != hipSuccess) return e;
    void* args[] = {&a};
    return hipLaunchKernel(k.fn, dim3(rl.G), dim3(k.threads), args, k.lds, c.stream);
}

}

extern "C" int fos_debug_res_stamps(long long* out, int n) {
#ifdef FOS_RES_STAMPS
    if (n > 4 * 16 * 64 * 16) n = 4 * 16 * 64 * 16;
    return (int)hipMemcpyFromSymbol(out, HIP_SYMBOL(fos::g_res_stamps), sizeof(long long) * (size_t)n);
#else
    (void)out; (void)n; return -1;
#endif
}
```

### firstordersolvers.jl_amd/csrc/solver.cpp

```cpp
#include <dlfcn.h>
#include <functional>

#include <chrono>
#include <cmath>
#include <mutex>

#include "fos_solver.hpp"

namespace fos {
const char* last_error_cstr();

struct Roctx {
    int state = 0;
    int (*push)(const char*) = nullptr;
    int (*pop)() = nullptr;
};
static Roctx g_roctx;
static bool roctx_on() {
    if (g_roctx.state == 0) {
        g_roctx.state = -1;
        const char* e = getenv("FOS_ROCTX");
        if (e && atoi(e) != 0) {
            const char* names[] = {"librocprofiler-sdk-roctx.so", "librocprofiler-sdk-roctx.so.1", "libroctx64.so", "libroctx64.so.4"};
            for (const char* nm : names) {
// ... 125 lines not shown
}

}

using namespace fos;

namespace {

int wait_cg_mark(fos_solver* h, uint32_t epoch, int32_t batch_id, bool* ended) {
    FOS_TRY(check_launch("poll"));
    volatile HostMark* m = h->mark;
    static const double wait_s = getenv("FOS_CG_WAIT_S") ? atof(getenv("FOS_CG_WAIT_S")) : 120.0;
    const auto t0 = std::chrono::steady_clock::now();
    for (uint32_t spin = 1;; ++spin) {
        if (__atomic_load_n(&m->seq, __ATOMIC_ACQUIRE) == epoch) { *ended = true; break; }
        if (__atomic_load_n(&m->batch, __ATOMIC_ACQUIRE) == batch_id) { *ended = false; break; }
        __builtin_ia32_pause();
        if ((spin & 0xFFFFu) == 0 && hipStreamQuery(h->stream) == hipSuccess) {
            if (__atomic_load_n(&m->seq, __ATOMIC_ACQUIRE) == epoch) { *ended = true; break; }
            if (__atomic_load_n(&m->batch, __ATOMIC_ACQUIRE) == batch_id) { *ended = false; break; }
            FOS_TRY(poll_state(h));
            *ended = h->st_host->done != 0;
            return FOS_OK;
        }
        if ((spin & 0xFFFFFu) == 0 && std::chrono::duration<double>(std::chrono::steady_clock::now() - t0).count() > wait_s) {
            set_error("CG solve %u: neither its end mark nor its batch mark arrived within %.0f s (a kernel of the solve does not finish)", epoch, wait_s);
            return FOS_EHIP;
        }
    }
    if (*ended) { h->st_host->done = 1; h->st_host->iter = m->iter; h->st_host->hit_max = m->hit_max; h->st_host->rr = m->rr; }
    else h->st_host->done = 0;
    return FOS_OK;
}

typedef std::function<int(const LaunchCtx&)> PostFn;
int cg_solve(fos_solver* h, d2* x, const d2* rhs, double tol, int maxit, int64_t* iters, const d2* apply_on = nullptr,
             const PostFn* post = nullptr, bool* post_ran = nullptr) {
    LaunchCtx c = h->ctx();
    int next_j = 1;
    const bool fold = h->tr.peer_on && peer_fold_env();
    const bool rccl = h->sharded() && !fold;
    int32_t variant = FOS_CG_REFERENCE;
    FOS_TRY(fos_get_cg_variant(h, &variant));
    const bool resident = variant == FOS_CG_RESIDENT;
    const bool merged = variant == FOS_CG_MERGED_SWEEP || variant == FOS_CG_MERGED_UPDATE;
    const bool close_in_update = variant == FOS_CG_MERGED_UPDATE;
    const bool fuse_p = variant == FOS_CG_FUSED_P;
    static const bool start_env = !(getenv("FOS_CG_FUSED_START") && atoi(getenv("FOS_CG_FUSED_START")) == 0);
    const bool start_fused = !merged && !h->sharded() && !c.between && start_env;
    const uint32_t nwin = (uint32_t)std::min<int64_t>((2 * (int64_t)std::max(maxit, 0) + 4 + 2047) / 2048, (int64_t)1 << 20);
    uint32_t epoch = h->cg_epoch + 1u;
    if (const uint32_t off = epoch & 0x1FFFFFu; off != 0u && off + (nwin - 1u) > 0x1FFFFFu) epoch += 0x200000u - off;
    h->cg_epoch = epoch + (nwin - 1u);
    const uint32_t seq_base = (uint32_t)(epoch * 2048u);
    auto iter_desc = [&](int j) {
        CgIter it;
        it.j = j; it.r = h->R; it.p_prev = h->PB[(j - 1) & 1]; it.p_cur = h->PB[j & 1];
        it.fuse_p = fuse_p; it.rr_from_reduced = rccl ? 1 : 0; it.fold = fold ? &h->tr.peer : nullptr; it.seq_base = seq_base;
        it.start_fused = start_fused;
        return it;
    };
    auto merged_desc = [&](int j) {
        CgmIter it;
        it.j = j; it.x = x; it.r = h->R; it.p = h->PB[0]; it.s = h->PB[1]; it.w = h->AP;
        it.close_in_update = close_in_update; it.from_reduced = rccl ? 1 : 0; it.fold = fold ? &h->tr.peer : nullptr; it.seq_base = seq_base;
        return it;
    };
    const size_t prof_start = h->prof_used;
    const bool spec = post && h->speculate && !c.between && !fuse_p && (seq_base >> 11) != 0u &&
                      (!h->sharded() || (fold && h->alg != FOS_ALG_GAPA));
    const int32_t batch_id = (int32_t)(((seq_base >> 11) & 0x7FFFFFu) << 8 | 1u);
    bool mark_last = spec;
    auto merged_reduce = [&](int j) -> int {
        if (c.between) FOS_TRY(c.between(c.between_arg));
        if (!rccl) return FOS_OK;
        launch_reduce1(c, c.S.nwg, 3, 1, 0);
        LaunchCtx c2 = c;
        c2.partials = c.partials + 3 * (size_t)PART_CAP + (size_t)((j - 1) & 1) * CGM_RR_STRIDE;
        c2.reduced = c.reduced + 3;
        launch_reduce1(c2, c.cg_blocks, 1, 1);
        return allreduce(h, 4);
    };
    if (resident) {
        const int pe = prof_begin(h, FOS_PROF_RESIDENT, 1, h->prof_seen[FOS_PROF_RESIDENT]++);
        const hipError_t le = launch_cg_resident(c, h->op.res, x, rhs, apply_on ? apply_on : x, tol, maxit, fold ? &h->tr.peer : nullptr, seq_base);
        prof_end(h, pe);
        if (le != hipSuccess) { set_error("resident CG launch: %s", hipGetErrorString(le)); return FOS_EHIP; }
        if (spec) {
            LaunchCtx cg = c;
            cg.gate = &h->st->done;
            FOS_TRY((*post)(cg));
            bool ended = false;
            FOS_TRY(wait_cg_mark(h, (uint32_t)(seq_base >> 11), batch_id, &ended));
            if (!ended) { set_error("resident CG solve %u ended without its mark", (unsigned)(seq_base >> 11)); return FOS_EHIP; }
            if (post_ran) *post_ran = true;
        } else {
            FOS_TRY(poll_state(h));
            if (!h->st_host->done) { set_error("resident CG solve %u did not finish", (unsigned)(seq_base >> 11)); return FOS_EHIP; }
        }
        *iters = h->st_host->iter;
        h->cg_same_run = (h->st_host->iter == h->last_cg_pred) ? h->cg_same_run + 1 : 0;
        h->last_cg_pred = h->st_host->iter;
        h->cg_total += h->st_host->iter;
        if (h->st_host->hit_max) h->hit_max_accum = 1;
        return FOS_OK;
    }
    if (merged) {
        CgmIter it0 = merged_desc(0);
        const d2* v = apply_on ? apply_on : x;
        const int po = prof_begin_other(h, 0);
        launch_cgm_apply(c, it0, v);
        if (c.between) FOS_TRY(c.between(c.between_arg));
        if (rccl) { launch_reduce1(c, c.S.nwg, 3, 0, 0); FOS_TRY(allreduce(h, 3)); }
        launch_cgm_start(c, it0, rhs, v, tol, maxit);
        prof_end(h, po);
        const int pe = prof_begin(h, FOS_PROF_KKT, 0, h->cg_total);
        launch_cgm_sweep(c, it0, close_in_update ? -1 : 0);
        prof_end(h, pe);
    } else if (start_fused) {
        CgmIter it0 = merged_desc(0);
        const d2* v = apply_on ? apply_on : x;
        const int po = prof_begin_other(h, 0);
        launch_cgm_apply(c, it0, v);
        launch_cgm_start(c, it0, rhs, v, tol, maxit, h->PB[1]);
        prof_end(h, po);
    } else {
        int fr = 0;
        const int po = prof_begin_other(h, 0);
        FOS_TRY(kkt_apply_full(h, c, apply_on ? apply_on : x, h->AP));
        launch_cg_init(c, rhs, h->AP, h->R, h->PB[1]);
        FOS_TRY(finish_reduce(h, c, c.vec_blocks, 1, 0, &fr));
        launch_cg_init_finalize(c, h->R, tol, maxit, fr);
        prof_end(h, po);
    }
    auto enqueue = [&](int count) -> int {
        if (merged) {
            for (int q = 0; q < count && next_j <= maxit; ++q, ++next_j) {
                CgmIter it = merged_desc(next_j);
                const bool last = q == count - 1 || next_j == maxit;
                if (mark_last && last) it.batch_mark = batch_id;
                FOS_TRY(merged_reduce(next_j));
                int pe = prof_begin(h, FOS_PROF_CGVEC, next_j, (h->cg_total + next_j - 1) % 4 == 1 ? (h->cg_total + next_j - 1) / 4 : 1);
                launch_cgm_update(c, it, false);
                prof_end(h, pe);
                pe = prof_begin(h, FOS_PROF_KKT, next_j + (close_in_update ? 0 : 1), h->cg_total + next_j);
                launch_cgm_sweep(c, it, close_in_update ? -1 : next_j);
                prof_end(h, pe);
            }
            if (close_in_update) {
                CgmIter it = merged_desc(next_j);
                if (mark_last) it.batch_mark = batch_id;
                FOS_TRY(merged_reduce(next_j));
                launch_cgm_update(c, it, true);
            }
            return FOS_OK;
        }
        for (int q = 0; q < count && next_j <= maxit; ++q, ++next_j) {
            CgIter it = iter_desc(next_j);
            if (mark_last && (q == count - 1 || next_j == maxit)) it.batch_mark = batch_id;
            int pe = prof_begin(h, FOS_PROF_KKT, next_j, h->cg_total + next_j - 1);
            launch_kkt2_cg(c, it, h->AP);
            prof_end(h, pe);
            int f1 = 0;
            if (c.between) FOS_TRY(c.between(c.between_arg));
            if (rccl) { launch_reduce1(c, c.S.nwg, 3, 1, 0); FOS_TRY(allreduce(h, 3)); f1 = 1; }
            pe = prof_begin(h, FOS_PROF_CGVEC, next_j, (h->cg_total + next_j - 1) % 4 == 1 ? (h->cg_total + next_j - 1) / 4 : 1);
// ... 635 lines not shown
    FOS_HIP(hipMemcpyAsync(lp.nu, nu2.data(), sizeof(double) * 2 * K, hipMemcpyHostToDevice, c.stream));
    launch_long_apply(c, X, lp.P, K, lp.nu);
    FOS_HIP(hipStreamSynchronize(c.stream));
    lp.log[0] = (double)i; lp.log[1] = (double)best_active; lp.log[2] = (double)best_viol; lp.log[3] = (double)qsqrt(step2 > 0 ? step2 : (qreal)0);
    lp.log[4] = (double)K; lp.log[5] = (double)tried;
    return FOS_OK;
}
void long_save_plane(const LaunchCtx& c, LongPlanes& lp, int which, const d2* y, const d2* x) {
    const int64_t row = 2 * (lp.savepos - 1) + which;
    launch_long_plane(c, lp.P + row * c.l, x, y, lp.bpart + row * c.vec_blocks);
}
}

extern "C" {

int fos_abi_version(void) { return FOS_ABI_VERSION; }
const char* fos_last_error(void) { return fos::last_error_cstr(); }

int fos_device_count(int* count) {
    int n = 0;
    hipError_t e = hipGetDeviceCount(&n);
    if (e != hipSuccess || n <= 0) {
        if (count) *count = 0;
        set_error("no HIP device visible (%s): libfoship has no CPU fallback", e == hipSuccess ? "count = 0" : hipGetErrorString(e));
        return FOS_ENODEVICE;
    }
    if (count) *count = n;
    return FOS_OK;
}

int fos_device_name(int device, char* buf, int buflen) {
    hipDeviceProp_t prop;
    FOS_HIP(hipGetDeviceProperties(&prop, device));
    snprintf(buf, buflen, "%s (%s, %d CUs)", prop.name, prop.gcnArchName, prop.multiProcessorCount);
    return FOS_OK;
}

struct HandleGuard {
    fos_solver* h;
    ~HandleGuard() { if (h) fos_destroy(h); }
};

int fos_create(int64_t m, int64_t n, const int64_t* colptr, const int64_t* rowval, const double* nzval,
               const double* b, const double* c,
               int64_t nK1, const int32_t* K1type, const int64_t* K1start, const int64_t* K1len,
               int64_t nK2, const int32_t* K2type, const int64_t* K2start, const int64_t* K2len,
               int device, fos_handle* out) {
    return fos_create2(m, n, colptr, rowval, nzval, b, c, nK1, K1type, K1start, K1len, nK2, K2type, K2start, K2len, device, 0, out);
}

int fos_create2(int64_t m, int64_t n, const int64_t* colptr, const int64_t* rowval, const double* nzval,
                const double* b, const double* c,
                int64_t nK1, const int32_t* K1type, const int64_t* K1start, const int64_t* K1len,
                int64_t nK2, const int32_t* K2type, const int64_t* K2start, const int64_t* K2len,
                int device, int32_t flags, fos_handle* out) {
    if (!out) { set_error("out handle is NULL"); return FOS_EINVAL; }
    *out = nullptr;
    if (m < 0 || n < 0 || !colptr || (!rowval && colptr[n] > 1) || (!b && m) || (!c && n)) { set_error("NULL or negative argument"); return FOS_EINVAL; }
    int ndev = 0;
    FOS_TRY(fos_device_count(&ndev));
    if (device < 0 || device >= ndev) { set_error("device %d out of range (0..%d)", device, ndev - 1); return FOS_EINVAL; }
    FOS_TRY(cone_table_check("K1", m, nK1, K1type, K1start, K1len));
    FOS_TRY(cone_table_check("K2", n, nK2, K2type, K2start, K2len));
    FOS_HIP(hipSetDevice(device));

    HandleGuard guard{new fos_solver()};
    fos_solver* h = guard.h;
    h->device = device;
    h->m = m; h->n = n; h->l = n + m + 1; h->l_global = h->l;
    h->nnz = colptr[n] - 1;
    FOS_HIP(hipStreamCreateWithFlags(&h->stream, hipStreamNonBlocking));
    FOS_HIP(hipHostMalloc((void**)&h->mark, sizeof(HostMark), hipHostMallocMapped));
    memset(h->mark, 0, sizeof(HostMark));
    h->speculate = !(getenv("FOS_SPECULATE") && atoi(getenv("FOS_SPECULATE")) == 0);
    h->shift_fuse = !(getenv("FOS_SHIFT_FUSE") && atoi(getenv("FOS_SHIFT_FUSE")) == 0);

    hipDeviceProp_t prop;
    FOS_HIP(hipGetDeviceProperties(&prop, device));
    const int cus = prop.multiProcessorCount > 0 ? prop.multiProcessorCount : 256;
    h->cus = cus;
    const PsdTuning psd_tuning = PsdTuning::from_env();
    h->psd_fuse = !(getenv("FOS_PSD_FUSE") && atoi(getenv("FOS_PSD_FUSE")) == 0);
    h->relax_ew = !(getenv("FOS_RELAX_EW") && atoi(getenv("FOS_RELAX_EW")) == 0);

    h->row_sharded = (flags & FOS_CREATE_ROW_SHARDED) != 0;
    FOS_TRY(operator_setup(h, colptr, rowval, nzval));
    h->fuse_p = false;
    if (const char* e = getenv("FOS_CG_FUSE_P")) h->fuse_p = atoi(e) != 0;
    if (const char* e = getenv("FOS_CG_VARIANT")) h->cg_variant = std::max(-1, std::min((int)FOS_CG_RESIDENT, atoi(e)));

    std::vector<double> cbv((size_t)(n + m));
    for (int64_t j = 0; j < n; ++j) { cbv[j] = c[j]; }
    for (int64_t i = 0; i < m; ++i) { cbv[n + i] = b[i]; }
    h->nb = std::sqrt(sum_squares(b, m)); h->nc = std::sqrt(sum_squares(c, n));
    h->nb_local = h->nb; h->nc_local = h->nc;
    FOS_TRY(dev_upload(h, &h->cb, cbv));

    const size_t l = (size_t)h->l;
    d2** vecs[] = {&h->X, &h->T1, &h->T2, &h->SOL, &h->RHS, &h->R, &h->PB[0], &h->PB[1], &h->AP, &h->Y, &h->XOLD, &h->W, &h->SOL2};
    for (d2** v : vecs) FOS_TRY(dev_zeros(h, v, l));
    FOS_TRY(dev_alloc(h, &h->plain, 2 * l));
    h->vec_blocks = (int)std::max<int64_t>(1, std::min<int64_t>((h->l + 255) / 256, 1024));
    h->cg_blocks = std::min(h->vec_blocks, getenv("FOS_CG_BLOCKS") ? std::max(1, atoi(getenv("FOS_CG_BLOCKS"))) : 2 * cus);
    if (h->op.dev.ndef > 0)
        h->cg_blocks = std::max<int>(h->cg_blocks, (int)std::min<int64_t>(1024, ((int64_t)h->op.dev.ndef * h->op.dev.def_lpr + 255) / 256));
    h->cg_blocks = std::min(h->cg_blocks, 1024);

    ConeTable table;
    table.ew.assign(l, 0);
    cone_table_add(table, 0, CONE_K2, nK2, K2type, K2start, K2len);
    cone_table_add(table, n, CONE_K1, nK1, K1type, K1start, K1len);
    table.ew[l - 1] = (uint8_t)(EW_MAX0 | (EW_MAX0 << 2));
    ConeSetOptions cone_opts;
    cone_opts.warm = !getenv("FOS_PSD_COLD");
    cone_opts.refine_records = true;
    cone_opts.debug_rec = getenv("FOS_PSD_DEBUG_REC") != nullptr;
    FOS_TRY(cone_set_build(table, (int64_t)l, cone_opts, psd_tuning, &h->cones));

    FOS_TRY(dev_zeros(h, &h->st, 1));
    FOS_TRY(dev_zeros(h, &h->pre_sums, 128));
    h->pre_on = !(getenv("FOS_CG_PRE") && atoi(getenv("FOS_CG_PRE")) == 0);
    {
        void* dp = nullptr;
        FOS_HIP(hipHostGetDevicePointer(&dp, h->mark, 0));
        const unsigned long long addr = (unsigned long long)(uintptr_t)dp;
        FOS_HIP(hipMemcpy(&h->st->hostmark, &addr, sizeof(addr), hipMemcpyHostToDevice));
    }
    FOS_HIP(hipHostMalloc((void**)&h->st_host, sizeof(DevState), hipHostMallocDefault));
    memset(h->st_host, 0, sizeof(DevState));
    FOS_TRY(dev_alloc(h, &h->partials, (size_t)6 * PART_CAP));
    FOS_TRY(dev_zeros(h, &h->reduced, 16));
    if (const char* e = getenv("FOS_CG_CHUNK")) h->cg_chunk = std::max(1, atoi(e));

    FOS_TRY(resident_setup(h, cus));
    FOS_TRY(fos_set_alg(h, FOS_ALG_GAP, 0.8, 1.8, 1.8, 0.0));
    FOS_TRY(fos_set_iterate(h, nullptr));
    FOS_HIP(hipStreamSynchronize(h->stream));
    *out = h;
    guard.h = nullptr;
    return FOS_OK;
}

int fos_create3(int64_t m, int64_t n, const int64_t* colptr, const int64_t* rowval, const double* nzval,
                const double* b, const double* c,
                int64_t nK1, const int32_t* K1type, const int64_t* K1start, const int64_t* K1len,
                int64_t nK2, const int32_t* K2type, const int64_t* K2start, const int64_t* K2len,
                int device, int32_t flags, int32_t equil_passes, fos_handle* out) {
    if (equil_passes == 0) return fos_create2(m, n, colptr, rowval, nzval, b, c, nK1, K1type, K1start, K1len, nK2, K2type, K2start, K2len, device, flags, out);
    if (!out) { set_error("out handle is NULL"); return FOS_EINVAL; }
    *out = nullptr;
    if (equil_passes < 0 || equil_passes > EQ_MAX_PASSES) { set_error("equil_passes = %d: 0 .. %d", (int)equil_passes, EQ_MAX_PASSES); return FOS_EINVAL; }
    if (flags & FOS_CREATE_ROW_SHARDED) {
        set_error("equilibration needs the whole problem on one handle: a rank knows neither the other ranks' column norms nor the global sigma, rho");
        return FOS_EUNSUPPORTED;
    }
    EqScaling eq;
    FOS_TRY(host_equilibrate(m, n, colptr, rowval, nzval, b, c, nK1, K1type, K1start, K1len, nK2, K2type, K2start, K2len, equil_passes, &eq));
    fos_handle h = nullptr;
    FOS_TRY(fos_create2(m, n, colptr, rowval, eq.nz.data(), eq.b.data(), eq.c.data(), nK1, K1type, K1start, K1len, nK2, K2type, K2start, K2len, device, flags, &h));
    HandleGuard guard{h};
    h->eq_nb = std::sqrt(sum_squares(b, m)); h->eq_nc = std::sqrt(sum_squares(c, n));
    h->eq_sigma = eq.sigma; h->eq_rho = eq.rho; h->eq_gamma = eq.gamma;
    const size_t l = (size_t)h->l;
    std::vector<d2> up(l);
    std::vector<double> inv((size_t)(n + m)), cbv((size_t)(n + m));
    for (int64_t j = 0; j < n; ++j) {
        up[j] = make_double2(eq.sigma / eq.E[j], eq.rho * eq.E[j]);
        inv[j] = 1.0 / eq.E[j];
        cbv[j] = eq.c[j];
    }
    for (int64_t i = 0; i < m; ++i) {
        up[n + i] = make_double2(eq.rho / eq.D[i], eq.sigma * eq.D[i]);
        inv[n + i] = 1.0 / eq.D[i];
        cbv[n + i] = eq.b[i];
    }
    up[l - 1] = make_double2(1.0, eq.sigma * eq.rho);
    for (const d2& u : up)
        if (!(u.x > 0.0) || !(u.y > 0.0) || !std::isfinite(u.x) || !std::isfinite(u.y)) { set_error("equilibration: a scale factor left the range of fp64"); return FOS_EINVAL; }
    FOS_TRY(dev_upload(h, &h->eq_up, up));
    FOS_TRY(dev_upload(h, &h->eq_inv, inv));
    FOS_TRY(dev_upload(h, &h->eq_cb, cbv));
    FOS_TRY(dev_zeros(h, &h->eq_w, l));
    h->eq_D.swap(eq.D);
    h->eq_E.swap(eq.E);
    h->eq_passes = equil_passes;
    *out = h;
    guard.h = nullptr;
    return FOS_OK;
}

int fos_get_equilibration(fos_handle h, int32_t* passes, double* D, double* E, double* scal3) {
    if (!h) { set_error("NULL handle"); return FOS_EINVAL; }
    if (passes) *passes = h->eq_passes;
    if (D) { if (h->equilibrated()) std::copy(h->eq_D.begin(), h->eq_D.end(), D); else std::fill(D, D + h->m, 1.0); }
    if (E) { if (h->equilibrated()) std::copy(h->eq_E.begin(), h->eq_E.end(), E); else std::fill(E, E + h->n, 1.0); }
    if (scal3) { scal3[0] = h->eq_sigma; scal3[1] = h->eq_rho; scal3[2] = h->eq_gamma; }
    return FOS_OK;
}

int fos_destroy(fos_handle h) {
    if (!h) return FOS_OK;
    (void)hipSetDevice(h->device);
    if (h->stream) (void)hipStreamSynchronize(h->stream);
    transport_teardown(h, true);
    for (auto& r : h->prof_recs) { (void)hipEventDestroy(r.a); (void)hipEventDestroy(r.b); }
    cone_set_destroy(h->cones, h->stream);
    for (void* p : h->pooled) uncached_release(p);
    for (void* p : h->owned) (void)hipFree(p);
    if (h->st_host) (void)hipHostFree(h->st_host);
    if (h->mark) (void)hipHostFree(h->mark);
    if (h->stream) (void)hipStreamDestroy(h->stream);
    delete h;
    return FOS_OK;
}

int fos_sizes(fos_handle h, int64_t* m, int64_t* n, int64_t* N, int64_t* nnz) {
    if (!h) { set_error("NULL handle"); return FOS_EINVAL; }
// ... 418 lines not shown
            launch_cgm_apply(c, it, h->W);
            launch_cgm_start(c, it, h->RHS, h->W, -1.0, INT32_MAX);
            launch_cgm_sweep(c, it, it.close_in_update ? -1 : 0);
            for (int j = 1; j <= iters; ++j) {
                it.j = j;
                launch_cgm_update(c, it, false);
                launch_cgm_sweep(c, it, it.close_in_update ? -1 : j);
            }
            return;
        }
        for (int j = 1; j <= iters; ++j) {
            CgIter it;
            it.j = j; it.r = h->R; it.p_prev = h->PB[(j - 1) & 1]; it.p_cur = h->PB[j & 1];
            it.fuse_p = variant == FOS_CG_FUSED_P; it.rr_from_reduced = 0; it.fold = nullptr; it.seq_base = seq_base;
            launch_kkt2_cg(c, it, h->AP);
            launch_cg_update(c, it, h->W, h->R, h->AP, 0);
            if (!it.fuse_p) launch_cg_pupdate(c, it, h->W, h->PB[(j + 1) & 1]);
        }
    };
    hipEvent_t e0, e1;
    FOS_HIP(hipEventCreate(&e0));
    FOS_HIP(hipEventCreate(&e1));
    hipGraph_t graph = nullptr;
    hipGraphExec_t exec = nullptr;
    if (use_graph) {
        FOS_HIP(hipStreamSynchronize(h->stream));
        FOS_HIP(hipStreamBeginCapture(h->stream, hipStreamCaptureModeThreadLocal));
        chain();
        FOS_HIP(hipStreamEndCapture(h->stream, &graph));
        FOS_HIP(hipGraphInstantiate(&exec, graph, nullptr, nullptr, 0));
        FOS_HIP(hipGraphLaunch(exec, h->stream));
    } else {
        chain();
    }
    FOS_HIP(hipEventRecord(e0, h->stream));
    for (int rep = 0; rep < reps; ++rep) {
        if (use_graph) FOS_HIP(hipGraphLaunch(exec, h->stream));
        else chain();
    }
    FOS_HIP(hipEventRecord(e1, h->stream));
    FOS_HIP(hipEventSynchronize(e1));
    float ms = 0.f;
    FOS_HIP(hipEventElapsedTime(&ms, e0, e1));
    *ms_per_iter = (double)ms / ((double)reps * iters);
    if (exec) (void)hipGraphExecDestroy(exec);
    if (graph) (void)hipGraphDestroy(graph);
    (void)hipEventDestroy(e0);
    (void)hipEventDestroy(e1);
    FOS_TRY(check_launch("fos_bench_cg_chain"));
    FOS_TRY(poll_state(h));
    return FOS_OK;
}

int fos_sync(fos_handle h) {
    if (!h) { set_error("NULL handle"); return FOS_EINVAL; }
    FOS_HIP(hipSetDevice(h->device));
    FOS_HIP(hipStreamSynchronize(h->stream));
    return FOS_OK;
}

static int refuse_fused_p_on_window_panels(const fos_solver* h) {
    if (h->op.dev.npanel == 0) return FOS_OK;
    set_error("FOS_CG_FUSED_P: the operator is stored in window panels, whose sweeps cannot build p on the fly (row-block and tile storage only)");
    return FOS_EUNSUPPORTED;
}

int fos_set_tuning(fos_handle h, int32_t spmv_workgroups, int32_t cg_chunk, int32_t fuse_p) {
    if (!h) { set_error("NULL handle"); return FOS_EINVAL; }
    FOS_HIP(hipSetDevice(h->device));
    if (fuse_p > 0) FOS_TRY(refuse_fused_p_on_window_panels(h));
    if (fuse_p >= 0) { h->fuse_p = fuse_p != 0; h->cg_variant = -1; }
    if (cg_chunk > 0) h->cg_chunk = cg_chunk;
    if (spmv_workgroups > 0) FOS_TRY(operator_repartition(h, spmv_workgroups));
    return FOS_OK;
}

int fos_set_cg_variant(fos_handle h, int32_t variant) {
    if (!h || variant < -1 || variant > FOS_CG_RESIDENT) { set_error("unknown CG variant %d", (int)variant); return FOS_EINVAL; }
    if (variant == FOS_CG_RESIDENT && !h->op.res_ok) {
        set_error("FOS_CG_RESIDENT: the operator does not qualify (%s)", h->op.res_plan.why.empty() ? "no plan" : h->op.res_plan.why.c_str());
        return FOS_EUNSUPPORTED;
    }
    if (variant == FOS_CG_FUSED_P) FOS_TRY(refuse_fused_p_on_window_panels(h));
    h->cg_variant = variant;
    if (variant >= 0) h->fuse_p = variant == FOS_CG_FUSED_P;
    h->last_cg_pred = 0; h->cg_same_run = 0;
    return FOS_OK;
}

int fos_get_cg_variant(fos_handle h, int32_t* variant) {
    if (!h || !variant) { set_error("NULL argument"); return FOS_EINVAL; }
    const bool fold_env = peer_fold_env();
    int v = h->cg_variant >= 0 ? h->cg_variant
            : (h->fuse_p ? FOS_CG_FUSED_P : ((h->sharded() || (h->op.dev.resident && !h->row_sharded && h->l >= 32768)) ? FOS_CG_MERGED_UPDATE : FOS_CG_REFERENCE));
    const bool res_default = !(getenv("FOS_RESIDENT_DEFAULT") && atoi(getenv("FOS_RESIDENT_DEFAULT")) == 0);
    const bool res_usable = h->op.res_ok && !h->row_sharded && (!h->sharded() || (h->tr.peer_on && fold_env && h->op.res_all));
    if (h->cg_variant < 0 && !h->fuse_p && h->sharded() && res_usable && res_default) v = FOS_CG_RESIDENT;
    if (h->cg_variant < 0 && !h->fuse_p && !h->sharded() && res_usable && res_default && h->op.res_plan.stream && 2 * h->op.res_plan.G >= h->cus) v = FOS_CG_RESIDENT;
    if (v == FOS_CG_RESIDENT && !res_usable) v = FOS_CG_MERGED_UPDATE;
    if (v == FOS_CG_FUSED_P && h->op.dev.npanel > 0) v = FOS_CG_REFERENCE;
    if (v == FOS_CG_MERGED_SWEEP && h->sharded()) v = FOS_CG_MERGED_UPDATE;
    if (v == FOS_CG_MERGED_UPDATE && h->tr.peer_on && !fold_env) v = FOS_CG_REFERENCE;
    *variant = v;
    return FOS_OK;
}

int fos_debug_set(fos_handle h, int32_t what, int64_t value) {
    if (!h) { set_error("NULL handle"); return FOS_EINVAL; }
    FOS_HIP(hipSetDevice(h->device));
    if (what == FOS_DEBUG_PUPDATE_DELAY) {
        const int32_t v = (int32_t)std::max<int64_t>(0, std::min<int64_t>(value, 100000000));
        FOS_HIP(hipStreamSynchronize(h->stream));
        FOS_HIP(hipMemcpy(&h->st->dbg_delay, &v, sizeof(v), hipMemcpyHostToDevice));
        return FOS_OK;
    }
    set_error("unknown debug switch %d", (int)what);
    return FOS_EINVAL;
}

}
```

### firstordersolvers.jl_amd/interface.py

```python
from __future__ import annotations

import ctypes as C
import time

import math

import numpy as np
import scipy.sparse as sp

from . import _lib

HEADER_CG = " Iter | pri res | dua res | rel gap | pri obj | dua obj | kap/tau | cg  | time"
HEADER_DIRECT = " Iter | pri res | dua res | rel gap | pri obj | dua obj | kap/tau | time"



class FOSAlgorithm:
    direct = False
    options: dict

    def _alg_args(self):
        raise NotImplementedError


# ... 301 lines not shown
        return v.value

    def alpha12(self):
        v = C.c_double(0)
        _lib.check(self._lib.fos_get_alpha12(self._h, C.byref(v)))
        return v.value

    def prox_count(self):
        v = C.c_int64(0)
        _lib.check(self._lib.fos_get_prox_count(self._h, C.byref(v)))
        return v.value

    def q_apply(self, x, transpose=False):
        x = _lib.as_f64(x, self.l)
        y = np.empty(self.l)
        _lib.check(self._lib.fos_q_apply(self._h, _lib.dptr(y), _lib.dptr(x), 1 if transpose else 0))
        return y

    def kkt_apply(self, x):
        x = _lib.as_f64(x, self.N)
        y = np.empty(self.N)
        _lib.check(self._lib.fos_kkt_apply(self._h, _lib.dptr(y), _lib.dptr(x)))
        return y

    def cg_kkt(self, x0, rhs, tol, max_iters=10000):
        x = _lib.as_f64(x0, self.N).copy()
        rhs = _lib.as_f64(rhs, self.N)
        it = C.c_int64(0)
        _lib.check(self._lib.fos_cg_kkt(self._h, _lib.dptr(x), _lib.dptr(rhs), tol, max_iters, C.byref(it)))
        return x, it.value

    def prox_affine(self, x):
        x = _lib.as_f64(x, self.N)
        y = np.empty(self.N)
        _lib.check(self._lib.fos_prox_affine(self._h, _lib.dptr(y), _lib.dptr(x)))
        return y

    def hsdematrix_prox(self, x):
        x = _lib.as_f64(x, self.N)
        y = np.empty(self.N)
        _lib.check(self._lib.fos_hsdematrix_prox(self._h, _lib.dptr(y), _lib.dptr(x)))
        return y

    def prox_cones(self, x):
        x = _lib.as_f64(x, self.N)
        y = np.empty(self.N)
        _lib.check(self._lib.fos_prox_cones(self._h, _lib.dptr(y), _lib.dptr(x)))
        return y

    def check(self, z, eps=1e-5):
        z = _lib.as_f64(z, self.N)
        res = _lib.CheckResult()
        _lib.check(self._lib.fos_check(self._h, _lib.dptr(z), eps, C.byref(res)))
        return res

    def profile(self, enable):
        _lib.check(self._lib.fos_profile(self._h, int(enable)))

    def profile_read(self):
        n = C.c_int64(0)
        ms = C.c_double(0)
        by = C.c_double(0)
        _lib.check(self._lib.fos_profile_read(self._h, C.byref(n), C.byref(ms), C.byref(by)))
        return n.value, ms.value, by.value

    def bench_kkt(self, reps):
        ms = C.c_double(0)
        _lib.check(self._lib.fos_bench_kkt(self._h, reps, C.byref(ms)))
        return ms.value

    def cg_total(self):
        v = C.c_int64(0)
        _lib.check(self._lib.fos_get_cg_total(self._h, C.byref(v)))
        return v.value

    def operator_stats(self):
        st = (C.c_int64 * 12)()
        _lib.check(self._lib.fos_operator_stats(self._h, st))
        keys = ("blocks", "ell", "lds", "long", "run", "vals", "cols", "waves", "tiles", "slots", "deferred", "tile_vals")
        out = dict(zip(keys, list(st)))
        ws = (C.c_int64 * 4)()
        _lib.check(self._lib.fos_window_stats(self._h, ws))
        out.update(zip(("win_panels", "win_segments", "win_slices", "win_vals"), list(ws)))
        return out

    def sync(self):
        _lib.check(self._lib.fos_sync(self._h))

    DIRECT_FORMS = {"auto": 0, "reduced": 4}

    def enable_direct(self, A, form="auto", factor="newton"):
        if form not in self.DIRECT_FORMS:
            raise ValueError("direct form must be one of %s, not %r" % (sorted(self.DIRECT_FORMS), form))
        factor_code = direct_factor_code(factor)
        A = sp.csc_matrix(A)
        A.sort_indices()
        colptr = (A.indptr.astype(np.int64) + 1)
        rowval = (A.indices.astype(np.int64) + 1)
        nz = np.ascontiguousarray(A.data, dtype=np.float64)
        i64 = lambda a: a.ctypes.data_as(C.POINTER(C.c_int64))
        _lib.check(self._lib.fos_enable_direct3(self._h, i64(colptr), i64(rowval), _lib.dptr(nz), self.DIRECT_FORMS[form], factor_code))

    def disable_direct(self):
        _lib.check(self._lib.fos_disable_direct(self._h))

    def direct_mode(self):
        v = C.c_int32(0)
        _lib.check(self._lib.fos_get_direct_mode(self._h, C.byref(v)))
        return ("off", "dense", "block", "cg", "reduced")[v.value]

    def direct_stats(self):
        out = np.zeros(8)
        _lib.check(self._lib.fos_get_direct_stats2(self._h, _lib.dptr(out)))
        return {"form": ("off", "dense", "block", "cg", "reduced")[int(out[0])], "k": int(out[1]), "setup_s": float(out[2]), "ns_steps": int(out[3]),
                "factor": DIRECT_FACTOR_NAMES[int(out[4])], "invert_s": float(out[5]), "probe_resid": float(out[6]), "fell_back": int(out[7])}

    def set_tuning(self, spmv_workgroups=0, cg_chunk=0, fuse_p=-1):
        _lib.check(self._lib.fos_set_tuning(self._h, spmv_workgroups, cg_chunk, fuse_p))

    def set_cg_variant(self, variant):
        codes = {None: -1, "default": -1, "reference": _lib.CG_REFERENCE, "fused_p": _lib.CG_FUSED_P,
                 "merged_sweep": _lib.CG_MERGED_SWEEP, "merged_update": _lib.CG_MERGED_UPDATE, "resident": _lib.CG_RESIDENT}
        _lib.check(self._lib.fos_set_cg_variant(self._h, codes[variant] if not isinstance(variant, int) else variant))

    def cg_variant_name(self):
        v = C.c_int32(0)
        _lib.check(self._lib.fos_get_cg_variant(self._h, C.byref(v)))
        return ("reference", "fused_p", "merged_sweep", "merged_update", "resident")[v.value]

    def resident_stats(self):
        st = (C.c_int64 * 8)()
        _lib.check(self._lib.fos_resident_stats(self._h, st))
        keys = ("qualifies", "workgroups", "waves_per_workgroup", "tiles_per_wave", "units", "max_tiles_per_workgroup", "steps_per_tile", "all_ranks_qualify")
        out = {k: int(st[i]) for i, k in enumerate(keys)}
        out["form"] = "streamed" if out["tiles_per_wave"] < 0 else "registers"
        out["tiles_per_wave"] = abs(out["tiles_per_wave"])
        return out

    def debug_set(self, what, value):
        _lib.check(self._lib.fos_debug_set(self._h, int(what), int(value)))

    def profile_read_classes(self):
        n = (C.c_int64 * 5)()
        ms = (C.c_double * 5)()
        _lib.check(self._lib.fos_profile_read_classes(self._h, n, ms))
        return {k: (n[i], ms[i]) for i, k in enumerate(("kkt", "psd", "cgvec", "other", "resident"))}

    def psd_debug(self, collect_stats=True, phase_limit=0):
        _lib.check(self._lib.fos_psd_debug(self._h, 1 if collect_stats else 0, int(phase_limit)))

    def psd_sweeps(self):
        n = C.c_int64(0)
        _lib.check(self._lib.fos_psd_stats(self._h, None, 0, C.byref(n)))
        out = np.zeros(max(1, n.value), dtype=np.int32)
        _lib.check(self._lib.fos_psd_stats(self._h, out.ctypes.data_as(C.POINTER(C.c_int32)), n.value, C.byref(n)))
        return out[:n.value]

    def psd_fused_steps(self):
        v = C.c_int64(0)
        _lib.check(self._lib.fos_psd_fused_steps(self._h, C.byref(v)))
        return v.value

    def bench_cg_chain(self, iters, reps=5, use_graph=False):
        ms = C.c_double(0)
        _lib.check(self._lib.fos_bench_cg_chain(self._h, iters, reps, 1 if use_graph else 0, C.byref(ms)))
        return ms.value

    @staticmethod
    def comm_unique_id():
        buf = (C.c_ubyte * 128)()
        _lib.check(_lib.load().fos_comm_get_unique_id(buf))
        return bytes(buf)

    def comm_init(self, nranks, rank, unique_id: bytes):
        buf = (C.c_ubyte * 128).from_buffer_copy(unique_id)
        _lib.check(self._lib.fos_comm_init(self._h, nranks, rank, buf))

    def comm_init_host(self, nranks, rank, allreduce_sum):
        def _cb(user, buf, count):
            try:
                allreduce_sum(np.ctypeslib.as_array(buf, shape=(count,)))
                return 0
            except Exception:
                import traceback
                traceback.print_exc()
                return 1
        self._host_cb = _lib.ALLREDUCE_FN(_cb)
        _lib.check(self._lib.fos_comm_init_host(self._h, nranks, rank, C.cast(self._host_cb, C.c_void_p), None))

    def peer_export(self) -> bytes:
        buf = (C.c_ubyte * 64)()
        _lib.check(self._lib.fos_peer_export(self._h, buf))
        return bytes(buf)

    def peer_open(self, nranks, rank, handles, timeout_s=0.0):
        blob = b"".join(handles)
        assert len(blob) == 64 * nranks
        buf = (C.c_ubyte * len(blob)).from_buffer_copy(blob)
        _lib.check(self._lib.fos_peer_open(self._h, nranks, rank, buf, float(timeout_s)))

    def peer_open_host(self, nranks, rank, shm_name, timeout_s=0.0):
        _lib.check(self._lib.fos_peer_open_host(self._h, nranks, rank, shm_name.encode(), float(timeout_s)))

    def peer_close(self):
        _lib.check(self._lib.fos_peer_close(self._h))

    def peer_vec_export(self) -> bytes:
        buf = (C.c_ubyte * 64)()
        _lib.check(self._lib.fos_peer_vec_export(self._h, buf))
        return bytes(buf)

    def peer_vec_open(self, handles):
        blob = b"".join(handles)
        buf = (C.c_ubyte * len(blob)).from_buffer_copy(blob)
        _lib.check(self._lib.fos_peer_vec_open(self._h, buf))

    def peer_selftest(self, rounds=32) -> bool:
        ok = C.c_int32(0)
        _lib.check(self._lib.fos_peer_selftest(self._h, rounds, C.byref(ok)))
        return bool(ok.value)
# ... 905 lines not shown
```

### include/foship.h

```cpp
#ifndef FOSHIP_H
#define FOSHIP_H

#include <stdint.h>

#ifdef __cplusplus
extern "C" {
#endif

#define FOS_ABI_VERSION 1

#define FOS_OK            0
#define FOS_EINVAL       -1
#define FOS_EHIP         -2
#define FOS_ENOMEM       -3
#define FOS_EUNSUPPORTED -4
#define FOS_ECOMM        -5
#define FOS_ENODEVICE    -6

#define FOS_CONE_FREE       0
#define FOS_CONE_ZERO       1
#define FOS_CONE_NONNEG     2
#define FOS_CONE_NONPOS     3
#define FOS_CONE_SOC        4
#define FOS_CONE_SOCROT     5
// ... 87 lines not shown
#define FOS_DIRECT_FORM_AUTO 0
#define FOS_DIRECT_FORM_REDUCED 4
int fos_enable_direct2(fos_handle h, const int64_t* colptr, const int64_t* rowval, const double* nzval, int32_t form);
int fos_get_direct_stats(fos_handle h, double* out4);
#define FOS_DIRECT_FACTOR_NEWTON 0
#define FOS_DIRECT_FACTOR_CHOLESKY 1
int fos_enable_direct3(fos_handle h, const int64_t* colptr, const int64_t* rowval, const double* nzval, int32_t form, int32_t factor);
int fos_get_direct_stats2(fos_handle h, double* out8);
int fos_dense_spd_inverse(int32_t device, int64_t k, const double* K, double* X, int32_t factor, double* info4);
int fos_host_chol_inverse(int64_t k, const double* K, double* X, int64_t* bad_pivot);
int fos_host_reduced_symm(int64_t k, const double* X, const double* pq, double* y, int32_t* count);

int fos_set_iterate(fos_handle h, const double* z);
int fos_get_iterate(fos_handle h, double* z);
int fos_get_checked(fos_handle h, double* z);

int fos_step(fos_handle h, int64_t i_first, int64_t count, int64_t checki, double eps,
             int64_t* iters_done, int32_t* checked, fos_check_result* res);

int fos_set_linesearch(fos_handle h, int64_t lsinterval);
int fos_linesearch_log(fos_handle h, double* out34);
int fos_set_longstep(fos_handle h, int64_t longinterval, int64_t nsave);
int fos_longstep_log(fos_handle h, double* out8);
int fos_set_gapp(fos_handle h, int64_t iproj);
int fos_gapp_log(fos_handle h, double* out23);

int fos_getsol(fos_handle h, double* z_out, int32_t force_check, double eps, fos_check_result* res);

int fos_get_affine_state(fos_handle h, double* xinit, int64_t* i, int32_t* firstrun);
int fos_set_affine_state(fos_handle h, const double* xinit, int64_t i);

int fos_get_alg_state(fos_handle h, double* a, double* b, double* scal2);
int fos_set_alg_state(fos_handle h, const double* a, const double* b, const double* scal2);

int fos_get_cgiter(fos_handle h, int64_t* cgiter);
int fos_get_alpha12(fos_handle h, double* alpha12);
int fos_get_prox_count(fos_handle h, int64_t* i);

int fos_q_apply(fos_handle h, double* y, const double* x, int32_t transpose);
int fos_kkt_apply(fos_handle h, double* y, const double* x);
int fos_cg_kkt(fos_handle h, double* x, const double* rhs, double tol, int64_t max_iters, int64_t* iters);
int fos_prox_affine(fos_handle h, double* y, const double* x);
int fos_hsdematrix_prox(fos_handle h, double* y, const double* x);
int fos_prox_cones(fos_handle h, double* y, const double* x);
int fos_check(fos_handle h, const double* z, double eps, fos_check_result* res);

int fos_operator_stats(fos_handle h, int64_t* stats12);
int fos_window_stats(fos_handle h, int64_t* stats4);
int fos_profile(fos_handle h, int32_t enable);
int fos_get_cg_total(fos_handle h, int64_t* total);
int fos_profile_read(fos_handle h, int64_t* launches, double* total_ms, double* bytes_per_launch);
#define FOS_PROF_KKT 0
#define FOS_PROF_PSD 1
#define FOS_PROF_CGVEC 2
#define FOS_PROF_OTHER 3
#define FOS_PROF_RESIDENT 4
#define FOS_PROF_CLASSES 5
int fos_profile_read_classes(fos_handle h, int64_t* launches5, double* total_ms5);
int fos_bench_cg_chain(fos_handle h, int32_t iters, int32_t reps, int32_t use_graph, double* ms_per_iter);
int fos_bench_kkt(fos_handle h, int32_t reps, double* total_ms);
int fos_psd_debug(fos_handle h, int32_t collect_stats, int32_t phase_limit);
int fos_psd_stats(fos_handle h, int32_t* sweeps, int64_t cap, int64_t* count);
int fos_psd_fused_steps(fos_handle h, int64_t* count);
int fos_sync(fos_handle h);

int fos_host_stacked_spmv(int64_t m, int64_t n, const int64_t* colptr, const int64_t* rowval, const double* nzval,
                          const double* v, double* out, int32_t spmv_workgroups, int32_t resident_waves, int64_t* stats);
int fos_host_resident_cg(int64_t m, int64_t n, const int64_t* colptr, const int64_t* rowval, const double* nzval, const double* b, const double* c,
                         int32_t gmax, double* x, const double* rhs, double tol, int64_t max_iters, int64_t* iters, int64_t* stats8);
int fos_host_resident_plan(int64_t m, int64_t n, const int64_t* colptr, const int64_t* rowval, const double* nzval, int32_t gmax,
                           int64_t* info8, int32_t* wg7, int64_t wg_cap, int64_t* tile5, int64_t tile_cap);
int fos_host_stacked_spmv_mode(int64_t m, int64_t n, const int64_t* colptr, const int64_t* rowval, const double* nzval,
                               const double* v, double* out, int32_t window_mode, int64_t* stats16);

int fos_set_tuning(fos_handle h, int32_t spmv_workgroups, int32_t cg_chunk, int32_t fuse_p);

#define FOS_CG_REFERENCE     0
#define FOS_CG_FUSED_P       1
#define FOS_CG_MERGED_SWEEP  2
#define FOS_CG_MERGED_UPDATE 3
#define FOS_CG_RESIDENT      4
int fos_set_cg_variant(fos_handle h, int32_t variant);
int fos_resident_stats(fos_handle h, int64_t* stats8);
int fos_get_cg_variant(fos_handle h, int32_t* variant);

#define FOS_DEBUG_PUPDATE_DELAY 1
int fos_debug_set(fos_handle h, int32_t what, int64_t value);

typedef struct fos_feas* fos_feas_handle;
int fos_feas_create(int64_t n, int32_t device, fos_feas_handle* out);
int fos_feas_destroy(fos_feas_handle h);
int fos_feas_set_affine(fos_feas_handle h, int32_t which, int64_t m, const double* A, const double* b);
int fos_feas_set_affine_sparse(fos_feas_handle h, int32_t which, int64_t m, const int64_t* colptr, const int64_t* rowval, const double* nzval, const double* b);
int fos_feas_affine_stats(fos_feas_handle h, int32_t which, double* out8);
int fos_feas_set_affine_factored(fos_feas_handle h, int32_t which, int64_t m, const double* A, const double* b, int32_t factor, int32_t refine);
int fos_feas_affine_factored_stats(fos_feas_handle h, int32_t which, double* out8);
int fos_feas_affine_factored_plan(fos_feas_handle h, int32_t which, int64_t* out6);
int fos_host_affine_factored(int64_t m, int64_t n, const double* A, const double* b, int32_t refine, const double* x, double* y);
int fos_feas_set_least_squares(fos_feas_handle h, int32_t which, int64_t m, const double* A, const double* b, double lambda, int32_t factor);
int fos_host_least_squares(int64_t m, int64_t n, const double* A, const double* b, double lambda, const double* x, double* y);
int fos_feas_set_affine_sparse_factored(fos_feas_handle h, int32_t which, int64_t m, const int64_t* colptr, const int64_t* rowval,
                                        const double* nzval, const double* b, int32_t factor, int32_t refine);
int fos_feas_affine_sparse_factored_stats(fos_feas_handle h, int32_t which, double* out8);
int fos_feas_affine_sparse_factored_plan(fos_feas_handle h, int32_t which, int64_t* out8);
int fos_host_affine_sparse_factored(int64_t m, int64_t n, const int64_t* colptr, const int64_t* rowval, const double* nzval, const double* b,
                                    int32_t refine, const double* x, double* y);
#define FOS_LS_FORM_SPARSE_FACTORED 0
#define FOS_LS_FORM_NORMAL 1
int fos_feas_set_quadratic(fos_feas_handle h, int32_t which, const double* Q, const double* q, int32_t factor);
int fos_feas_set_least_squares_normal(fos_feas_handle h, int32_t which, int64_t m, const double* A, const double* b, double lambda, int32_t factor);
int fos_feas_set_least_squares_sparse(fos_feas_handle h, int32_t which, int64_t m, const int64_t* colptr, const int64_t* rowval, const double* nzval,
                                      const double* b, double lambda, int32_t form, int32_t factor);
int fos_feas_nspace_stats(fos_feas_handle h, int32_t which, double* out8);
int fos_host_quadratic(int64_t n, const double* Q, const double* q, const double* x, double* y);
int fos_host_least_squares_normal(int64_t m, int64_t n, const double* A, const double* b, double lambda, const double* x, double* y);
int fos_host_least_squares_sparse(int64_t m, int64_t n, const int64_t* colptr, const int64_t* rowval, const double* nzval, const double* b, double lambda,
                                  int32_t form, const double* x, double* y);
int fos_host_symv_packed(int64_t k, const double* X, const double* v, double* y, int32_t* count);
int fos_feas_set_quadratic_sparse(fos_feas_handle h, int32_t which, const int64_t* colptr, const int64_t* rowval, const double* nzval, const double* q, double tol);
int fos_feas_set_least_squares_cg(fos_feas_handle h, int32_t which, int64_t m, const int64_t* colptr, const int64_t* rowval, const double* nzval, const double* b,
                                  double lambda, double tol);
int fos_feas_nspace_cg_stats(fos_feas_handle h, int32_t which, double* out8);
int fos_host_quadratic_cg(int64_t n, const int64_t* colptr, const int64_t* rowval, const double* nzval, const double* q, double tol, const double* x, double* y,
                          int32_t* iters);
int fos_host_least_squares_cg(int64_t m, int64_t n, const int64_t* colptr, const int64_t* rowval, const double* nzval, const double* b, double lambda, double tol,
                              const double* x, double* y, int32_t* iters);
int fos_bench_symv_packed(int32_t device, int64_t k, int32_t reps, double* out4);
int fos_feas_set_box(fos_feas_handle h, int32_t which, double lo, double hi);
int fos_feas_set_box_arrays(fos_feas_handle h, int32_t which, const double* lo, const double* hi);
int fos_feas_set_cones(fos_feas_handle h, int32_t which, int64_t ncones, const int32_t* type, const int64_t* len);
typedef int32_t (*fos_prox_fn)(void* ctx, int64_t n, const double* x, double* y);
int fos_feas_set_callback(fos_feas_handle h, int32_t which, fos_prox_fn fn, void* ctx);
#define FOS_SET_FREE       0
#define FOS_SET_BALL_L2    1
#define FOS_SET_BALL_L1    2
#define FOS_SET_SIMPLEX    3
#define FOS_SET_HALFSPACE  4
#define FOS_SET_HYPERSLAB  5
#define FOS_SET_POINT      6
#define FOS_SET_BOX        7
#define FOS_FN_NORM_L1     32
#define FOS_FN_SQR_NORM_L2 33
#define FOS_FN_ELASTIC_NET 34
#define FOS_FN_LINEAR      35
#define FOS_FN_NORM_L2     36
#define FOS_FN_HUBER       37
#define FOS_FN_NORM_LINF   38
int fos_feas_set_blocks(fos_feas_handle h, int32_t which, int64_t nblocks, const int32_t* kind, const int64_t* len, const double* scal, const double* vec);
int fos_feas_set_stats(fos_feas_handle h, int32_t which, double* out8);
int fos_host_set_project(int32_t kind, int64_t len, const double* scal2, const double* vec, const double* x, double* y, int32_t* passes);
int fos_feas_set_alg(fos_feas_handle h, int32_t alg, double alpha, double alpha1, double alpha2, double beta);
int fos_feas_set_gapp(fos_feas_handle h, double alpha, double alpha1, double alpha2, int64_t iproj);
int fos_feas_gapp_log(fos_feas_handle h, double* out23);
int fos_feas_set_linesearch(fos_feas_handle h, int64_t lsinterval);
int fos_feas_set_longstep(fos_feas_handle h, int64_t longinterval, int64_t nsave);
int fos_feas_longstep_log(fos_feas_handle h, double* out8);
int fos_feas_linesearch_log(fos_feas_handle h, double* out34);
int fos_feas_set_iterate(fos_feas_handle h, const double* x0);
int fos_feas_step(fos_feas_handle h, int64_t first_iter, int64_t niter, int64_t checki, double eps, int64_t* done, int32_t* status, double* err,
                  int32_t* checked);
int fos_feas_getsol(fos_feas_handle h, double* sol, int32_t force_check, double eps, int32_t* status, double* err);
int fos_feas_get_iterate(fos_feas_handle h, double* x);
int fos_feas_prox(fos_feas_handle h, int32_t which, const double* x, double* y);
int fos_feas_info(fos_feas_handle h, double* alpha12, int32_t* ns_iters, double* ns_resid);

#ifdef __cplusplus
// ... 4 lines not shown
```

Measured before the change: 1186.

## Add adaptive fp32 matrix values to resident streamed CG SpMV

Adds a float32 copy of the SpMV matrix values and an error-bounded mixed-precision mode in the resident streamed CG kernel. A setup kernel computes a per-block rounding-error norm bound. The kernel switches to fp32 value loads once the residual is small enough, and reverts to fp64 when an accumulated error budget is exceeded. This halves the value bytes streamed from HBM per sweep during the low-precision phase. The cost is an extra one-time setup pass, more kernel template instances, and a risk of accuracy loss or extra iterations.

```diff
diff --git a/firstordersolvers.jl_amd/_lib.py b/firstordersolvers.jl_amd/_lib.py
--- a/firstordersolvers.jl_amd/_lib.py
+++ b/firstordersolvers.jl_amd/_lib.py
@@ -122,6 +122,7 @@
     "fos_set_cg_variant": (C.c_int, [_h, C.c_int32]),
     "fos_get_cg_variant": (C.c_int, [_h, _i32p]),
     "fos_resident_stats": (C.c_int, [_h, _i64p]),
+    "fos_resident_lowp_stats": (C.c_int, [_h, _dp]),
     "fos_debug_set": (C.c_int, [_h, C.c_int32, C.c_int64]),
     "fos_set_gapp": (C.c_int, [_h, C.c_int64]),
     "fos_gapp_log": (C.c_int, [_h, _dp]),
diff --git a/firstordersolvers.jl_amd/csrc/fos_internal.hpp b/firstordersolvers.jl_amd/csrc/fos_internal.hpp
--- a/firstordersolvers.jl_amd/csrc/fos_internal.hpp
+++ b/firstordersolvers.jl_amd/csrc/fos_internal.hpp
@@ -350,7 +350,9 @@
     unsigned long long* grec;
     unsigned long long* crec;
     int64_t timeout_ticks;
-};
+    const float* val32; double lowp_delta, lowp_eta; int lowp_mode; double* lowp_out;
+};
+hipError_t launch_rs_lowp_setup(hipStream_t stream, const BlkDesc* blk, const double* val, int64_t nvals, const ResWG* wg, int G, float* val32, double* part);
 hipError_t launch_cg_resident(const LaunchCtx& c, const ResLaunch& rl, double2* x, const double2* rhs, const double2* v, double tol, int maxit,
                               const PeerBox* fold, uint32_t seq_base);
 bool res_lds_fits(const ResLaunch& rl, int device, std::string* why);
diff --git a/firstordersolvers.jl_amd/csrc/fos_solver.hpp b/firstordersolvers.jl_amd/csrc/fos_solver.hpp
--- a/firstordersolvers.jl_amd/csrc/fos_solver.hpp
+++ b/firstordersolvers.jl_amd/csrc/fos_solver.hpp
@@ -60,6 +60,9 @@
     bool res_ok = false;
     bool res_all = false;
     int res_gmax = 0;
+    float* res_val32 = nullptr;
+    bool res_lowp_pending = false;
+    double* res_lowp_out = nullptr;
 };
 
 struct fos_solver {
@@ -87,6 +90,8 @@
     int cus = 256;
     bool psd_fuse = true;
     bool relax_ew = true;
+    int rs_lowp = 1;
+    double rs_lowp_eta = 0.1;
 
     fos::DevState* st = nullptr;
     fos::DevState* st_host = nullptr;
@@ -220,6 +225,7 @@
 int operator_setup(fos_solver* h, const int64_t* colptr, const int64_t* rowval, const double* nzval);
 int operator_repartition(fos_solver* h, int nwg);
 int resident_setup(fos_solver* h, int gmax);
+int resident_lowp_ensure(fos_solver* h);
 int prox_affine_direct(fos_solver* h, const d2* x);
 
 struct Scratch {
diff --git a/firstordersolvers.jl_amd/csrc/operator.cpp b/firstordersolvers.jl_amd/csrc/operator.cpp
--- a/firstordersolvers.jl_amd/csrc/operator.cpp
+++ b/firstordersolvers.jl_amd/csrc/operator.cpp
@@ -183,6 +183,31 @@
     stats8[6] = p.tmax; stats8[7] = all ? 1 : 0;
 }
 
+int resident_lowp_ensure(fos_solver* h) {
+    Operator& o = h->op;
+    if (!o.res_lowp_pending) return FOS_OK;
+    o.res_lowp_pending = false;
+    if (!o.res_ok || !o.res_plan.stream || h->rs_lowp == 0 || h->sharded() || o.dev.nnz_padded <= 0) return FOS_OK;
+    const int G = o.res_plan.G;
+    if (!o.res_val32) {
+        FOS_TRY(dev_alloc(h, &o.res_val32, (size_t)o.dev.nnz_padded));
+        FOS_TRY(dev_zeros(h, &o.res_lowp_out, 4));
+    }
+    double* part = nullptr;
+    FOS_TRY(dev_alloc(h, &part, (size_t)G));
+    std::vector<double> hp((size_t)G);
+    hipError_t e = launch_rs_lowp_setup(h->stream, o.dev.blk, o.dev.val, o.dev.nnz_padded, o.res_wg, G, o.res_val32, part);
+    if (e == hipSuccess) e = hipMemcpyAsync(hp.data(), part, sizeof(double) * hp.size(), hipMemcpyDeviceToHost, h->stream);
+    if (e == hipSuccess) e = hipStreamSynchronize(h->stream);
+    dev_release(h, &part);
+    FOS_HIP(e);
+    double delta = 0.0;
+    for (double v : hp) delta = (v > delta || v != v) ? v : delta;
+    if (!(delta < std::numeric_limits<double>::infinity())) return FOS_OK;
+    o.res.val32 = o.res_val32; o.res.lowp_out = o.res_lowp_out; o.res.lowp_delta = delta * (1.0 + 0x1p-20); o.res.lowp_mode = h->rs_lowp;
+    return FOS_OK;
+}
+
 int resident_setup(fos_solver* h, int gmax) {
     Operator& o = h->op;
     if (const char* e = getenv("FOS_RESIDENT_GMAX")) gmax = std::max(1, std::min(gmax, atoi(e)));
@@ -214,6 +239,8 @@
     o.res = plan_launch(plan, o.res);
     static const double res_wait_s = getenv("FOS_RESIDENT_WAIT_S") ? atof(getenv("FOS_RESIDENT_WAIT_S")) : 5.0;
     o.res.timeout_ticks = (int64_t)(res_wait_s * 1e8);
+    o.res.val32 = nullptr; o.res.lowp_out = nullptr; o.res.lowp_delta = 0.0; o.res.lowp_eta = h->rs_lowp_eta; o.res.lowp_mode = 0;
+    o.res_lowp_pending = true;
     o.res_plan = plan; o.res_ok = true; o.res_all = !h->sharded();
     return FOS_OK;
 }
@@ -253,6 +280,19 @@
     const Operator& o = h->op;
     plan_stats8(o.res_plan, o.res_ok, h->sharded() ? o.res_all : o.res_ok, stats8);
     if (!o.res_ok) set_error("FOS_CG_RESIDENT: %s", o.res_plan.why.empty() ? "no plan" : o.res_plan.why.c_str());
+    return FOS_OK;
+}
+
+int fos_resident_lowp_stats(fos_handle h, double* stats8) {
+    if (!h || !stats8) { set_error("NULL argument"); return FOS_EINVAL; }
+    const Operator& o = h->op;
+    for (int k = 0; k < 8; ++k) stats8[k] = 0.0;
+    if (!o.res_ok || !o.res.val32) return FOS_OK;
+    double rec[4];
+    FOS_HIP(hipStreamSynchronize(h->stream));
+    FOS_HIP(hipMemcpy(rec, o.res.lowp_out, sizeof(rec), hipMemcpyDeviceToHost));
+    stats8[0] = o.res.lowp_delta; stats8[1] = rec[0]; stats8[2] = rec[1]; stats8[3] = rec[2];
+    stats8[4] = 4.0 * (double)o.dev.nnz_padded; stats8[5] = (double)o.res.lowp_mode; stats8[6] = o.res.lowp_eta;
     return FOS_OK;
 }
 
diff --git a/firstordersolvers.jl_amd/csrc/resident.hip b/firstordersolvers.jl_amd/csrc/resident.hip
--- a/firstordersolvers.jl_amd/csrc/resident.hip
+++ b/firstordersolvers.jl_amd/csrc/resident.hip
@@ -11,6 +11,7 @@
     DevState* st;
     const BlkDesc* blk;
     const double* val;
+    const float* val32;
     const ResWG* wg;
     int G;
     unsigned long long* grec;
@@ -23,6 +24,8 @@
     PeerBox pb;
     uint32_t seq_base;
     long long timeout_ticks;
+    double lowp_delta, lowp_theta, lowp_budget;
+    double* lowp_out;
 };
 
 __device__ __forceinline__ void res_st_word(unsigned long long* p, unsigned long long w) { __hip_atomic_store(p, w, __ATOMIC_RELAXED, __HIP_MEMORY_SCOPE_AGENT); }
@@ -83,7 +86,7 @@
 #define RES_STAMP_NEXT() do { } while (0)
 #endif
 
-enum ResCtl { RC_ALPHA = 0, RC_BETA, RC_GTX, RC_GTY, RC_STOP, RC_NEAR, RC_COUNT };
+enum ResCtl { RC_ALPHA = 0, RC_BETA, RC_GTX, RC_GTY, RC_STOP, RC_NEAR, RC_LOWP, RC_COUNT };
 
 __device__ __forceinline__ bool res_peer_fold4(const PeerBox& pb, uint32_t seq, double (&tot)[4], bool first, uint32_t* halves ) {
     const int lane = threadIdx.x & 63;
@@ -535,7 +538,8 @@
 #ifndef RS_XC
 #define RS_XC 2
 #endif
-__device__ __forceinline__ void res_tile_plain(const double (&val)[TILE_GROUP], const d2 g, const d2* __restrict__ gcol, d2& u, double (&a1)[TILE_GROUP],
+template <class VT>
+__device__ __forceinline__ void res_tile_plain(const VT (&val)[TILE_GROUP], const d2 g, const d2* __restrict__ gcol, d2& u, double (&a1)[TILE_GROUP],
                                                double (&a2)[TILE_GROUP]) {
 #pragma unroll
     for (int h = 0; h < TILE_GROUP / RS_XC; ++h) {
@@ -544,7 +548,7 @@
         for (int k = 0; k < RS_XC; ++k) xc[k] = gcol[RS_XC * h + k];
 #pragma unroll
         for (int k = 0; k < RS_XC; ++k) {
-            const double v = val[RS_XC * h + k];
+            const double v = (double)val[RS_XC * h + k];
             u.x += v * xc[k].x; u.y += v * xc[k].y;
             a1[RS_XC * h + k] += v * g.x; a2[RS_XC * h + k] += v * g.y;
         }
@@ -563,10 +567,14 @@
     return d;
 }
 
-__device__ __forceinline__ void rs_request(const ResArgs& a, int blk, int grp, int lane, double (&val)[TILE_GROUP]) {
+template <class VT> __device__ __forceinline__ const VT* rs_values(const ResArgs& a);
+template <> __device__ __forceinline__ const double* rs_values<double>(const ResArgs& a) { return a.val; }
+template <> __device__ __forceinline__ const float* rs_values<float>(const ResArgs& a) { return a.val32; }
+template <class VT>
+__device__ __forceinline__ void rs_request(const ResArgs& a, int blk, int grp, int lane, VT (&val)[TILE_GROUP]) {
     const BlkDesc d = rs_desc(a.blk, blk);
     const bool live = TILE_GROUP * grp < d.steps();
-    const double* __restrict__ vp = a.val + d.nnz0 + (live ? 64 * TILE_GROUP * grp : 0) + (live ? lane : 0);
+    const VT* __restrict__ vp = rs_values<VT>(a) + d.nnz0 + (live ? 64 * TILE_GROUP * grp : 0) + (live ? lane : 0);
 #pragma unroll
     for (int t = 0; t < TILE_GROUP; ++t) val[t] = __builtin_nontemporal_load(vp + 64 * t);
 }
@@ -596,9 +604,9 @@
     }
 }
 
-template <int Q, int NT, int D>
+template <int Q, int NT, int D, class VT>
 __device__ __forceinline__ void rs_group(const ResArgs& a, int bf, int cnt, int grp, int c0, int lane, const d2* __restrict__ s_gcol, d2* __restrict__ mycol,
-                                         RsRows<NT>& R, double (&val)[D][TILE_GROUP], double (&a1)[TILE_GROUP], double (&a2)[TILE_GROUP]) {
+                                         RsRows<NT>& R, VT (&val)[D][TILE_GROUP], double (&a1)[TILE_GROUP], double (&a2)[TILE_GROUP]) {
     if constexpr (Q < NT) {
         if (Q < cnt) {
             const BlkDesc d = rs_desc(a.blk, bf + Q);
@@ -615,7 +623,7 @@
 #pragma unroll
                 for (int u = 0; u < TILE_GROUP; ++u) a1[u] = a2[u] = 0.0;
             }
-            rs_group<Q + 1, NT, D>(a, bf, cnt, grp, c0, lane, s_gcol, mycol, R, val, a1, a2);
+            rs_group<Q + 1, NT, D, VT>(a, bf, cnt, grp, c0, lane, s_gcol, mycol, R, val, a1, a2);
         }
     }
 }
@@ -623,31 +631,41 @@
 #ifndef RS_RING
 #define RS_RING 2
 #endif
-template <int TMAX, int NT>
+template <int TMAX, int NT, class VT>
+__device__ __forceinline__ void rs_walk(const ResArgs& a, int blk_first, int cnt, int c0, int lane, const d2* __restrict__ s_gcol, d2* __restrict__ mycol,
+                                        RsRows<NT>& R) {
+    constexpr int RING = RS_RING * (int)(sizeof(double) / sizeof(VT));
+    constexpr int D = NT < RING ? NT : RING;
+    int tw = 0;
+#pragma unroll
+    for (int q = 0; q < NT; ++q) { const int t = rs_desc(a.blk, blk_first + (q < cnt ? q : cnt - 1)).steps(); tw = t > tw ? t : tw; }
+    const int ngrp = ((tw < TMAX ? tw : TMAX) + TILE_GROUP - 1) / TILE_GROUP;
+    VT val[D][TILE_GROUP];
+    double a1[TILE_GROUP], a2[TILE_GROUP];
+#pragma unroll
+    for (int s = 0; s < D; ++s) if (s < cnt) rs_request<VT>(a, blk_first + s, 0, lane, val[s]);
+#pragma unroll
+    for (int q = 0; q < NT; ++q) R.ww[q] = make_double2(0.0, 0.0);
+#pragma unroll
+    for (int u = 0; u < TILE_GROUP; ++u) a1[u] = a2[u] = 0.0;
+    for (int grp = 0; grp < ngrp; ++grp) {
+        int bf = blk_first;
+        asm volatile("" : "+s"(bf));
+        rs_group<0, NT, D, VT>(a, bf, cnt, grp, c0, lane, s_gcol, mycol, R, val, a1, a2);
+    }
+}
+template <int TMAX, int NT, bool LOWP>
 __device__ __forceinline__ void rs_sweep(const ResArgs& a, int blk_first, int cnt, int c0, int lane, const d2* __restrict__ s_gcol, const double* s_ctl,
                                          d2* __restrict__ mycol, RsRows<NT>& R, double (&acc)[4], bool early = false,
                                          const double* __restrict__ cbh = nullptr) {
-    constexpr int D = NT < RS_RING ? NT : RS_RING;
     if (early) cnt = 0;
     mycol[lane] = make_double2(0.0, 0.0);
     acc[0] = acc[1] = acc[2] = acc[3] = 0.0;
     if (cnt > 0) {
-        int tw = 0;
-#pragma unroll
-        for (int q = 0; q < NT; ++q) { const int t = rs_desc(a.blk, blk_first + (q < cnt ? q : cnt - 1)).steps(); tw = t > tw ? t : tw; }
-        const int ngrp = ((tw < TMAX ? tw : TMAX) + TILE_GROUP - 1) / TILE_GROUP;
-        double val[D][TILE_GROUP], a1[TILE_GROUP], a2[TILE_GROUP];
-#pragma unroll
-        for (int s = 0; s < D; ++s) if (s < cnt) rs_request(a, blk_first + s, 0, lane, val[s]);
-#pragma unroll
-        for (int q = 0; q < NT; ++q) R.ww[q] = make_double2(0.0, 0.0);
-#pragma unroll
-        for (int u = 0; u < TILE_GROUP; ++u) a1[u] = a2[u] = 0.0;
-        for (int grp = 0; grp < ngrp; ++grp) {
-            int bf = blk_first;
-            asm volatile("" : "+s"(bf));
-            rs_group<0, NT, D>(a, bf, cnt, grp, c0, lane, s_gcol, mycol, R, val, a1, a2);
-        }
+        bool lowp = false;
+        if constexpr (LOWP) lowp = __builtin_amdgcn_readfirstlane((int)(s_ctl[RC_LOWP] != 0.0)) != 0;
+        if (lowp) rs_walk<TMAX, NT, float>(a, blk_first, cnt, c0, lane, s_gcol, mycol, R);
+        else rs_walk<TMAX, NT, double>(a, blk_first, cnt, c0, lane, s_gcol, mycol, R);
         double cb[NT];
 #pragma unroll
         for (int q = 0; q < NT; ++q) {
@@ -763,7 +781,23 @@
     return !bad;
 }
 
-template <int TMAX, int NT>
+enum ResLowp { LP_STATE = 0, LP_PI, LP_BOUND, LP_SWEEPS, LP_COUNT };
+__device__ __forceinline__ double rs_lowp_decide(const ResArgs& a, double* s_lowp, int lane, bool start, bool cur, double gam, double alpha, double beta) {
+    if (a.val32 == nullptr) return 0.0;
+    double state = s_lowp[LP_STATE], pi = s_lowp[LP_PI], bound = s_lowp[LP_BOUND], sweeps = s_lowp[LP_SWEEPS];
+    if (start) { if (a.lowp_theta == INFINITY) state = 1.0; }
+    else {
+        if (cur) sweeps += 1.0;
+        pi = (cur ? gam : 0.0) + beta * beta * pi;
+        bound += a.lowp_delta * fabs(alpha) * sqrt(pi);
+        if (state == 1.0 && a.lowp_budget >= 0.0 && bound > a.lowp_budget) state = 2.0;
+        else if (state == 0.0 && sqrt(gam) <= a.lowp_theta) state = 1.0;
+    }
+    if (lane == 0) { s_lowp[LP_STATE] = state; s_lowp[LP_PI] = pi; s_lowp[LP_BOUND] = bound; s_lowp[LP_SWEEPS] = sweeps; }
+    return state == 1.0 ? 1.0 : 0.0;
+}
+
+template <int TMAX, int NT, bool LOWP>
 __global__ __launch_bounds__(64 * (RS_NCOMP + 1)) void cg_stream_kernel(ResArgs a) {
     __shared__ __attribute__((aligned(16))) d2 s_gcol[64];
     __shared__ double s_red[16][4];
@@ -771,6 +805,7 @@
     __shared__ uint32_t s_halves[PEER_MAX_RANKS * 8];
     __shared__ int s_cnt, s_failed;
     __shared__ double s_tau[9];
+    __shared__ double s_lowp[LP_COUNT];
     extern __shared__ __attribute__((aligned(16))) double s_dyn[];
     d2* const s_colpart = reinterpret_cast<d2*>(s_dyn);
     double* const s_all = reinterpret_cast<double*>(s_colpart + (RS_NCOMP + 1) * 64);
@@ -819,7 +854,7 @@
         bool early = false;
         for (int i = -1, xr = 0;; ++xr) {
             double acc[4];
-            rs_sweep<TMAX, NT>(a, me.blk0 + t0, cnt, c0, lane, s_gcol, s_ctl, mycol, R, acc, early, HOLD_CB ? cbh : nullptr);
+            rs_sweep<TMAX, NT, LOWP>(a, me.blk0 + t0, cnt, c0, lane, s_gcol, s_ctl, mycol, R, acc, early, HOLD_CB ? cbh : nullptr);
 #pragma unroll
             for (int k = 0; k < 4; ++k) {
                 const double v = wave_sum(acc[k]);
@@ -867,7 +902,8 @@
         if (lane < tc) { cr = a.v[c0 + lane]; cx = a.x[c0 + lane]; cc = a.cb[c0 + lane]; }
         s_gcol[lane] = cr;
         const d2 gt = a.v[nm], xt = a.x[nm];
-        if (lane == 0) { s_ctl[RC_GTX] = gt.x; s_ctl[RC_GTY] = gt.y; s_ctl[RC_STOP] = 0.0; }
+        if (lane == 0) { s_ctl[RC_GTX] = gt.x; s_ctl[RC_GTY] = gt.y; s_ctl[RC_STOP] = 0.0; if (LOWP) s_ctl[RC_LOWP] = 0.0; }
+        if (LOWP && lane == 0) { s_lowp[LP_STATE] = 0.0; s_lowp[LP_PI] = 0.0; s_lowp[LP_BOUND] = 0.0; s_lowp[LP_SWEEPS] = 0.0; }
         if (lane == 0) { s_tau[0] = xt.x; s_tau[1] = xt.y; s_tau[2] = s_tau[3] = s_tau[4] = s_tau[5] = s_tau[6] = s_tau[7] = s_tau[8] = 0.0; }
         if (blockIdx.x == 0 && lane == 0) { st->tol = a.tol; st->maxit = a.maxit; st->hit_max = 0; st->rn_old = 0.0; }
     }
@@ -883,7 +919,7 @@
         nx += 1;
         if (c0wave) {
             double racc[4];
-            rs_sweep<TMAX, NTC>(a, me.blk0 + t0, cnt, c0, lane, s_gcol, s_ctl, mycol, R, racc, early);
+            rs_sweep<TMAX, NTC, LOWP>(a, me.blk0 + t0, cnt, c0, lane, s_gcol, s_ctl, mycol, R, racc, early);
 #pragma unroll
             for (int k = 0; k < 4; ++k) {
                 const double v = wave_sum(racc[k]);
@@ -1001,7 +1037,7 @@
             const double q1 = ctot.x + gt.x * cc, q2 = ctot.y + gt.y * cc;
             const d2 cwv = make_double2(cr.x - q2, q1 - cr.y);
             const d2 wt = make_double2(gt.x + tot[3], -tot[2] - gt.y);
-            double stopf = failed ? 2.0 : 0.0, alpha = 0.0, beta = 0.0, near = 0.0;
+            double stopf = failed ? 2.0 : 0.0, alpha = 0.0, beta = 0.0, near = 0.0, lowp = 0.0;
             if (!failed && early) {
                 gam = tot[0] + (gt.x * gt.x + gt.y * gt.y);
                 if (i > 0 && (sqrt(gam) <= a.tol || i >= a.maxit)) { iter = i; stopf = 1.0; }
@@ -1009,6 +1045,7 @@
                 if (i < 0) {
                     cr = make_double2(crhs.x - cwv.x, crhs.y - cwv.y);
                     gt = make_double2(rhst.x - wt.x, rhst.y - wt.y);
+                    if constexpr (LOWP) lowp = rs_lowp_decide(a, s_lowp, lane, true, false, 0.0, 0.0, 0.0);
                 } else {
                     gam = tot[0] + (gt.x * gt.x + gt.y * gt.y);
                     if (i > 0 && (sqrt(gam) <= a.tol || i >= a.maxit)) { iter = i; stopf = 1.0; }
@@ -1020,6 +1057,7 @@
                             alpha = gam / (delta - beta * gam / a_prev);
                         }
                         g_prev = gam; a_prev = alpha;
+                        if constexpr (LOWP) lowp = rs_lowp_decide(a, s_lowp, lane, false, s_ctl[RC_LOWP] != 0.0, gam, alpha, beta);
                         auto upd = [&](const d2 wi, d2& ri, d2& pi, d2& si, d2& xi) {
                             if (i == 0) { pi = ri; si = wi; }
                             else {
@@ -1037,7 +1075,7 @@
             }
             if (stopf == 0.0 && !early) s_gcol[lane] = lane < tc ? cr : make_double2(0.0, 0.0);
             if (lane == 0) {
-                if (!early) { s_ctl[RC_ALPHA] = alpha; s_ctl[RC_BETA] = beta; s_ctl[RC_GTX] = gt.x; s_ctl[RC_GTY] = gt.y; s_ctl[RC_NEAR] = near; }
+                if (!early) { s_ctl[RC_ALPHA] = alpha; s_ctl[RC_BETA] = beta; s_ctl[RC_GTX] = gt.x; s_ctl[RC_GTY] = gt.y; s_ctl[RC_NEAR] = near; if (LOWP) s_ctl[RC_LOWP] = lowp; }
                 s_ctl[RC_STOP] = stopf;
                 s_tau[0] = xt.x; s_tau[1] = xt.y; s_tau[2] = pt.x; s_tau[3] = pt.y; s_tau[4] = stt.x; s_tau[5] = stt.y; s_tau[6] = g_prev; s_tau[7] = a_prev; s_tau[8] = gam;
             }
@@ -1060,6 +1098,7 @@
         if (ok) rs_rows_store<NTC>(a, me.blk0 + t0, cnt, lane, R);
         if (ok && leader && lane < tc) a.x[c0 + lane] = cx;
         if (blockIdx.x == 0 && lane == 0) {
+            if (LOWP && a.lowp_out) { a.lowp_out[0] = s_lowp[LP_SWEEPS]; a.lowp_out[1] = s_lowp[LP_STATE] == 2.0 ? 1.0 : 0.0; a.lowp_out[2] = s_lowp[LP_BOUND]; }
             if (ok) {
                 a.x[nm] = make_double2(s_tau[0], s_tau[1]);
                 const double gam = s_tau[8];
@@ -1074,17 +1113,17 @@
 }
 
 struct ResKernel { const void* fn; int threads; size_t lds; };
-static ResKernel res_kernel(const ResLaunch& rl) {
+static ResKernel res_kernel(const ResLaunch& rl, bool lowp = false) {
     auto k = [](auto kern, int threads, size_t lds) { return ResKernel{reinterpret_cast<const void*>(kern), threads, lds}; };
     if (rl.stream) {
         const int thr = 64 * (RS_NCOMP + 1);
         const size_t lds = res_stream_lds_bytes(rl.tiles_wg_max);
-        if (rl.tmax > 32 && rl.nt <= 3) return k(cg_stream_kernel<64, 3>, thr, lds);
-        if (rl.tmax > 32) return k(cg_stream_kernel<64, 5>, thr, lds);
-        if (rl.nt <= 3) return k(cg_stream_kernel<32, 3>, thr, lds);
-        if (rl.nt <= 5) return k(cg_stream_kernel<32, 5>, thr, lds);
-        if (rl.nt <= 9) return k(cg_stream_kernel<32, 9>, thr, lds);
-        return k(cg_stream_kernel<32, 10>, thr, lds);
+        if (rl.tmax > 32 && rl.nt <= 3) return lowp ? k(cg_stream_kernel<64, 3, true>, thr, lds) : k(cg_stream_kernel<64, 3, false>, thr, lds);
+        if (rl.tmax > 32) return lowp ? k(cg_stream_kernel<64, 5, true>, thr, lds) : k(cg_stream_kernel<64, 5, false>, thr, lds);
+        if (rl.nt <= 3) return lowp ? k(cg_stream_kernel<32, 3, true>, thr, lds) : k(cg_stream_kernel<32, 3, false>, thr, lds);
+        if (rl.nt <= 5) return lowp ? k(cg_stream_kernel<32, 5, true>, thr, lds) : k(cg_stream_kernel<32, 5, false>, thr, lds);
+        if (rl.nt <= 9) return lowp ? k(cg_stream_kernel<32, 9, true>, thr, lds) : k(cg_stream_kernel<32, 9, false>, thr, lds);
+        return lowp ? k(cg_stream_kernel<32, 10, true>, thr, lds) : k(cg_stream_kernel<32, 10, false>, thr, lds);
     }
     const int thr = 64 * (rl.nw + rl.ncomm);
     if (rl.tmax <= 32 && rl.rpt == 1) return k(cg_resident_kernel<32, 1, 768>, thr, res_reg_lds_bytes(12, 32));
@@ -1093,13 +1132,17 @@
     return k(cg_resident_kernel<64, 1, 512>, thr, res_reg_lds_bytes(8, 64));
 }
 
+static bool res_lds_fits_instance(const ResKernel& k, int device, std::string* why);
 static hipError_t res_lds_optin(const ResKernel& k) {
     if (k.lds > 48 * 1024) return hipFuncSetAttribute(k.fn, hipFuncAttributeMaxDynamicSharedMemorySize, (int)k.lds);
     return hipSuccess;
 }
 
 bool res_lds_fits(const ResLaunch& rl, int device, std::string* why) {
-    const ResKernel k = res_kernel(rl);
+    if (rl.stream && !res_lds_fits_instance(res_kernel(rl, true), device, why)) return false;
+    return res_lds_fits_instance(res_kernel(rl, false), device, why);
+}
+static bool res_lds_fits_instance(const ResKernel& k, int device, std::string* why) {
     hipFuncAttributes fa{};
     int cap = 0;
     char buf[192];
@@ -1134,11 +1177,78 @@
     a.ncomp = rl.nw;
     static const int res_flags = getenv("FOS_RES_FLAGS") ? atoi(getenv("FOS_RES_FLAGS")) : (2 << 8);
     a.flags = res_flags;
-    const ResKernel k = res_kernel(rl);
+    if (rl.stream && rl.val32 && rl.lowp_mode > 0 && !fold) {
+        constexpr double K = 8.0;
+        const double tol_lp = std::min(tol, (double)c.l * 2.220446049250313e-16);
+        a.val32 = rl.val32; a.lowp_out = rl.lowp_out; a.lowp_delta = rl.lowp_delta;
+        a.lowp_theta = (rl.lowp_mode == 2 || rl.lowp_delta == 0.0) ? INFINITY : rl.lowp_eta * tol_lp / (K * rl.lowp_delta);
+        a.lowp_budget = rl.lowp_mode == 2 ? -1.0 : 0.5 * rl.lowp_eta * tol_lp;
+    }
+    const ResKernel k = res_kernel(rl, a.val32 != nullptr);
     const hipError_t e = res_lds_optin(k);
     if (e != hipSuccess) return e;
     void* args[] = {&a};
     return hipLaunchKernel(k.fn, dim3(rl.G), dim3(k.threads), args, k.lds, c.stream);
+}
+
+__global__ __launch_bounds__(256) void rs_lowp_round_kernel(const double* __restrict__ val, float* __restrict__ val32, int64_t n) {
+    for (int64_t i = (int64_t)blockIdx.x * 256 + threadIdx.x; i < n; i += (int64_t)gridDim.x * 256) val32[i] = (float)val[i];
+}
+
+__global__ __launch_bounds__(256) void rs_lowp_delta_kernel(const BlkDesc* __restrict__ blk, const double* __restrict__ val, const ResWG* __restrict__ wg,
+                                                            double* __restrict__ part) {
+    __shared__ double s_d[64][65];
+    __shared__ double s_row[256];
+    const int tid = threadIdx.x;
+    const ResWG me = wg[blockIdx.x];
+    if (me.idx != 0) { if (tid == 0) part[blockIdx.x] = 0.0; return; }
+    const int j = tid >> 2, k0 = (tid & 3) * 16;
+    double acc[16];
+#pragma unroll
+    for (int k = 0; k < 16; ++k) acc[k] = 0.0;
+    for (int kk = 0; kk < me.wpu; ++kk) {
+        const ResWG w = wg[me.wg0 + kk];
+        for (int ti = 0; ti < w.nblk; ++ti) {
+            const BlkDesc d = blk[w.blk0 + ti];
+            const int coff = d.meta[0] - me.c0, steps = d.steps();
+            int any = 0;
+            for (int e = tid; e < 64 * 64; e += 256) {
+                const int c = e >> 6, r = e & 63, t = c - coff;
+                double dv = 0.0;
+                if (t >= 0 && t < steps) { const double v = val[d.nnz0 + 64 * (int64_t)t + r]; dv = v - (double)(float)v; }
+                s_d[c][r] = dv;
+                any |= dv != 0.0;
+            }
+            if (__syncthreads_or(any)) {
+                for (int r = 0; r < 64; ++r) {
+                    const double dj = s_d[j][r];
+#pragma unroll
+                    for (int k = 0; k < 16; ++k) acc[k] += dj * s_d[k0 + k][r];
+                }
+            }
+            __syncthreads();
+        }
+    }
+    double s = 0.0;
+#pragma unroll
+    for (int k = 0; k < 16; ++k) s += fabs(acc[k]);
+    s_row[tid] = s;
+    __syncthreads();
+    if (tid == 0) {
+        double mx = 0.0;
+        for (int q = 0; q < 64; ++q) {
+            const double rs = (s_row[4 * q] + s_row[4 * q + 1]) + (s_row[4 * q + 2] + s_row[4 * q + 3]);
+            mx = rs > mx || rs != rs ? rs : mx;
+        }
+        part[blockIdx.x] = sqrt(mx);
+    }
+}
+
+hipError_t launch_rs_lowp_setup(hipStream_t stream, const BlkDesc* blk, const double* val, int64_t nvals, const ResWG* wg, int G, float* val32, double* part) {
+    const int grid = (int)std::min<int64_t>(4096, (nvals + 255) / 256);
+    if (grid > 0) hipLaunchKernelGGL(rs_lowp_round_kernel, dim3(grid), dim3(256), 0, stream, val, val32, nvals);
+    hipLaunchKernelGGL(rs_lowp_delta_kernel, dim3(G), dim3(256), 0, stream, blk, val, wg, part);
+    return hipGetLastError();
 }
 
 }
diff --git a/firstordersolvers.jl_amd/csrc/solver.cpp b/firstordersolvers.jl_amd/csrc/solver.cpp
--- a/firstordersolvers.jl_amd/csrc/solver.cpp
+++ b/firstordersolvers.jl_amd/csrc/solver.cpp
@@ -231,6 +231,7 @@
         return allreduce(h, 4);
     };
     if (resident) {
+        FOS_TRY(resident_lowp_ensure(h));
         const int pe = prof_begin(h, FOS_PROF_RESIDENT, 1, h->prof_seen[FOS_PROF_RESIDENT]++);
         const hipError_t le = launch_cg_resident(c, h->op.res, x, rhs, apply_on ? apply_on : x, tol, maxit, fold ? &h->tr.peer : nullptr, seq_base);
         prof_end(h, pe);
@@ -1032,6 +1033,8 @@
     const PsdTuning psd_tuning = PsdTuning::from_env();
     h->psd_fuse = !(getenv("FOS_PSD_FUSE") && atoi(getenv("FOS_PSD_FUSE")) == 0);
     h->relax_ew = !(getenv("FOS_RELAX_EW") && atoi(getenv("FOS_RELAX_EW")) == 0);
+    if (const char* e = getenv("FOS_RS_LOWP")) h->rs_lowp = std::max(0, std::min(2, atoi(e)));
+    if (const char* e = getenv("FOS_RS_LOWP_ETA")) { const double eta = atof(e); if (eta > 0.0 && eta <= 1.0) h->rs_lowp_eta = eta; }
 
     h->row_sharded = (flags & FOS_CREATE_ROW_SHARDED) != 0;
     FOS_TRY(operator_setup(h, colptr, rowval, nzval));
@@ -1083,6 +1086,11 @@
     if (const char* e = getenv("FOS_CG_CHUNK")) h->cg_chunk = std::max(1, atoi(e));
 
     FOS_TRY(resident_setup(h, cus));
+    {
+        int32_t v = FOS_CG_REFERENCE;
+        FOS_TRY(fos_get_cg_variant(h, &v));
+        if (v == FOS_CG_RESIDENT) FOS_TRY(resident_lowp_ensure(h));
+    }
     FOS_TRY(fos_set_alg(h, FOS_ALG_GAP, 0.8, 1.8, 1.8, 0.0));
     FOS_TRY(fos_set_iterate(h, nullptr));
     FOS_HIP(hipStreamSynchronize(h->stream));
@@ -1667,6 +1675,7 @@
         return FOS_EUNSUPPORTED;
     }
     if (variant == FOS_CG_FUSED_P) FOS_TRY(refuse_fused_p_on_window_panels(h));
+    if (variant == FOS_CG_RESIDENT) { FOS_HIP(hipSetDevice(h->device)); FOS_TRY(resident_lowp_ensure(h)); }
     h->cg_variant = variant;
     if (variant >= 0) h->fuse_p = variant == FOS_CG_FUSED_P;
     h->last_cg_pred = 0; h->cg_same_run = 0;
diff --git a/firstordersolvers.jl_amd/interface.py b/firstordersolvers.jl_amd/interface.py
--- a/firstordersolvers.jl_amd/interface.py
+++ b/firstordersolvers.jl_amd/interface.py
@@ -407,6 +407,7 @@
         ws = (C.c_int64 * 4)()
         _lib.check(self._lib.fos_window_stats(self._h, ws))
         out.update(zip(("win_panels", "win_segments", "win_slices", "win_vals"), list(ws)))
+        out["lowp_val32_bytes"] = int(self._lowp_stats()[4])
         return out
 
     def sync(self):
@@ -460,7 +461,14 @@
         out = {k: int(st[i]) for i, k in enumerate(keys)}
         out["form"] = "streamed" if out["tiles_per_wave"] < 0 else "registers"
         out["tiles_per_wave"] = abs(out["tiles_per_wave"])
+        lp = self._lowp_stats()
+        out.update(lowp_delta=lp[0], lowp_sweeps_last_solve=int(lp[1]), lowp_reverted_last_solve=int(lp[2]), lowp_bound_last_solve=lp[3])
         return out
+
+    def _lowp_stats(self):
+        lp = np.zeros(8)
+        _lib.check(self._lib.fos_resident_lowp_stats(self._h, _lib.dptr(lp)))
+        return [float(v) for v in lp]
 
     def debug_set(self, what, value):
         _lib.check(self._lib.fos_debug_set(self._h, int(what), int(value)))
diff --git a/include/foship.h b/include/foship.h
--- a/include/foship.h
+++ b/include/foship.h
@@ -193,6 +193,7 @@
 #define FOS_CG_RESIDENT      4
 int fos_set_cg_variant(fos_handle h, int32_t variant);
 int fos_resident_stats(fos_handle h, int64_t* stats8);
+int fos_resident_lowp_stats(fos_handle h, double* stats8);
 int fos_get_cg_variant(fos_handle h, int32_t* variant);
 
 #define FOS_DEBUG_PUPDATE_DELAY 1
```

New measurement: 1414, median of 6. 1.19x the previous value.
